# pyamg/pyamg

Measured on AMD Instinct MI355X. Metric: vcycle_iterations_per_sec, higher is better.
Workload: dtype f64; 1 GPU; 3D 7-pt Poisson 256^3 (16.7M dof) SA V-cycle, symmetric Gauss-Seidel, fp64; key=c3, n=16777216, nnz=117047296, levels=5, cycle=V(1,1), graph=True, parallelism=1 GPU, gs_order=fast, full=False

## Files before the change

include/pyamg_amd.h:

```cpp
#ifndef PYAMG_AMD_H
#define PYAMG_AMD_H

#include <stddef.h>
#include <stdint.h>

#ifdef __cplusplus
extern "C" {
#endif

#define PAMG_OK              0
#define PAMG_E_ARG          -1
#define PAMG_E_UNSUPPORTED  -2
#define PAMG_E_NODEVICE     -3
#define PAMG_E_STATE        -4
#define PAMG_E_ALLOC        -5
#define PAMG_E_TIMEOUT      -6
#define PAMG_E_NOCONV       -8

#define PAMG_F64 0
#define PAMG_F32 1

typedef void *pamg_stream_t;
typedef void *pamg_event_t;
typedef struct pamg_matrix_s *pamg_matrix_t;
// ... 314 lines not shown
#define PAMG_TUNE_ZERO_MERGE 40
#define PAMG_TUNE_GS_CORRECTION 41
int pamg_matrix_tune(pamg_matrix_t A, int key, int value);
int pamg_matrix_value_codes(pamg_matrix_t A, int *n_values);
int pamg_matrix_row_patterns(pamg_matrix_t A, int *n_patterns);
int pamg_matrix_row_masks(pamg_matrix_t A, long long info[8]);
int pamg_matrix_autotune(pamg_matrix_t A, int allow_cap);
int pamg_matrix_gs_profile(pamg_matrix_t A, int which, long long *out, int64_t capacity, int64_t *count);
int pamg_matrix_tile_info(pamg_matrix_t A, int which, int64_t info[8]);
int pamg_matrix_lane_info(pamg_matrix_t A, int which, int64_t info[8]);
int pamg_matrix_lanem_info(pamg_matrix_t A, int which, int64_t info[20], double *growth);
int pamg_matrix_point_twin(pamg_matrix_t A, int *state);
int pamg_matrix_lanem_levels(pamg_matrix_t A, int which, int64_t *out, int64_t capacity, int64_t *count);
int pamg_matrix_kz_info(pamg_matrix_t A, int which, int64_t info[8]);
int pamg_matrix_line_info(pamg_matrix_t A, int which, int64_t info[8]);
int pamg_matrix_lane_profile(pamg_matrix_t A, int which, long long *out, int64_t capacity, int64_t *count);
int pamg_matrix_subset_rows(pamg_matrix_t A, const int32_t *rows, int nrows, pamg_matrix_t *sub);
int pamg_matrix_kaczmarz(pamg_matrix_t L, int nr, void *v, const void *b, const void *Dinv, double omega,
                         int sweep, int iterations, void *xout, pamg_stream_t s);
int pamg_matrix_jacobi_indexed(pamg_matrix_t sub, void *x, const void *b, double omega, void *work,
                               pamg_stream_t s);
int pamg_matrix_flow_error(pamg_matrix_t A, int *error);

#define PAMG_SPMV_SET      0
#define PAMG_SPMV_ACC      1
#define PAMG_SPMV_RESID    2
#define PAMG_SPMV_AXPBY    3
#define PAMG_SPMV_ACC_AXPBY 4
int pamg_matrix_spmv(pamg_matrix_t A, int mode, const void *x, const void *b_or_v, double c,
                     void *y, pamg_stream_t s);
int pamg_matrix_split_ranges(pamg_matrix_t A, int64_t n_owned_cols);
int pamg_matrix_spmv_part(pamg_matrix_t A, int part, int mode, const void *x, const void *b_or_v, double c, void *y,
                          pamg_stream_t stream);
int pamg_matrix_resid_sumsq(pamg_matrix_t A, const void *x, const void *b, double *out_sumsq,
                            pamg_stream_t s);

#define PAMG_FORWARD   0
#define PAMG_BACKWARD  1
#define PAMG_SYMMETRIC 2
int pamg_matrix_jacobi(pamg_matrix_t A, void *x, const void *b, void *work, double omega,
                       int iterations, pamg_stream_t s);
int pamg_matrix_jacobi_step(pamg_matrix_t A, const void *x_in, const void *b, void *x_out,
                            double omega, pamg_stream_t s);
int pamg_matrix_block_jacobi_step(pamg_matrix_t A, const void *Dinv, const void *x_in, const void *b, void *x_out,
                                  double omega, pamg_stream_t s);
int pamg_matrix_block_jacobi_indexed(pamg_matrix_t A, const void *Dinv, void *x, const void *b, const int32_t *idx,
                                     int64_t nidx, double omega, void *work, pamg_stream_t s);
int pamg_matrix_gauss_seidel(pamg_matrix_t A, void *x, const void *b, int sweep, double omega,
                             int iterations, pamg_stream_t s);
int pamg_matrix_gauss_seidel_x0(pamg_matrix_t A, void *x, const void *b, int sweep, double omega,
                                int iterations, int x_is_zero, pamg_stream_t s);
int pamg_matrix_sym_info(pamg_matrix_t A, int64_t info[9]);
int pamg_matrix_gauss_seidel_correction(pamg_matrix_t A, void *x, const void *b, void *r, int iterations, pamg_stream_t s);
int pamg_matrix_polynomial(pamg_matrix_t A, void *x, const void *b, void *work,
                           const double *coeffs, int ncoeffs, int iterations, int x_is_zero,
                           pamg_stream_t s);
int pamg_matrix_block_jacobi(pamg_matrix_t A, void *x, const void *b, void *work,
                             const void *Dinv, double omega, int iterations, pamg_stream_t s);
int pamg_matrix_block_gauss_seidel(pamg_matrix_t A, void *x, const void *b, const void *Dinv,
                                   int sweep, int iterations, pamg_stream_t s);

int pamg_dev_pinv_array(int dtype, void *AA, int64_t m, int n, int transA, pamg_stream_t s);

int pamg_dev_schwarz_blocks(int dtype, pamg_matrix_t A, int nsub, const int32_t *d_Sp, const int32_t *d_Sj, int32_t *d_Tp,
                            void *d_Tx, int64_t Tx_capacity, double rank_tol, int invert, pamg_stream_t s, int64_t info[4]);
int pamg_schwarz_blocks(int dtype, pamg_matrix_t A, int nsub, const int32_t *Sp, const int32_t *Sj, int32_t *Tp, void *Tx,
                        int64_t Tx_capacity, double rank_tol, int invert, int64_t info[4]);

int pamg_vec_sumsq(int dtype, int64_t n, const void *x, double *out_sumsq, pamg_stream_t s);
int pamg_vec_axpy(int dtype, int64_t n, double a, const void *x, void *y, pamg_stream_t s);
int pamg_vec_scale(int dtype, int64_t n, double a, const void *x, void *y, pamg_stream_t s);
int pamg_vec_mul(int dtype, int64_t n, const void *a, const void *b, void *y, pamg_stream_t s);
int pamg_vec_gather(int dtype, int64_t n, const int32_t *idx, const void *src, void *dst,
                    pamg_stream_t s);

int pamg_csr_renumber(int dtype, int64_t nrows, int64_t ncols, const int32_t *Ap, const int32_t *Aj, const void *Ax,
                      const int32_t *row_old_of_new, const int32_t *col_new_of_old, int32_t *Bp, int32_t *Bj, void *Bx);
int pamg_csr_row_argmax_abs(int dtype, int64_t nrows, const int32_t *Ap, const int32_t *Aj, const void *Ax, int32_t *out);
int pamg_csr_sort_rows(int dtype, int64_t nrows, const int32_t *Ap, int32_t *Aj, void *Ax, int block);
int pamg_host_cpus(int fresh);

#define PAMG_SMOOTH_NONE        0
#define PAMG_SMOOTH_JACOBI      1
#define PAMG_SMOOTH_GS          2
#define PAMG_SMOOTH_SOR         3
#define PAMG_SMOOTH_POLY        4
#define PAMG_SMOOTH_BLOCK_JACOBI 5
#define PAMG_SMOOTH_BLOCK_GS    6
#define PAMG_SMOOTH_CF_JACOBI   7
#define PAMG_SMOOTH_FC_JACOBI   8
#define PAMG_SMOOTH_GS_NE       9
#define PAMG_SMOOTH_GS_NR      10
#define PAMG_SMOOTH_JACOBI_NE  11
#define PAMG_SMOOTH_CF_BLOCK_JACOBI 12
#define PAMG_SMOOTH_FC_BLOCK_JACOBI 13
#define PAMG_SMOOTH_SCHWARZ    14
#define PAMG_SMOOTH_KRYLOV     15
#define PAMG_KRYLOV_CG    0
#define PAMG_KRYLOV_GMRES 1
#define PAMG_KRYLOV_CGNE  2
#define PAMG_KRYLOV_CGNR  3
#define PAMG_CYCLE_V 0
#define PAMG_CYCLE_W 1
#define PAMG_CYCLE_F 2
#define PAMG_CYCLE_AMLI 3
int pamg_solver_create(pamg_solver_t *S, int dtype);
// ... 121 lines not shown
```

pyamg_amd/_build.py:

```python
from __future__ import annotations

import os
import shutil
import subprocess
import sys
from concurrent.futures import ThreadPoolExecutor
from pathlib import Path

PKG = Path(__file__).resolve().parent
CSRC = PKG / "csrc"
LIB = PKG / "libpyamg_amd.so"
SOURCES = ["pamg_matrix.hip", "pamg_solver.hip", "pamg_capi.hip", "pamg_setup.hip", "pamg_schwarz.hip", "pamg_dist.hip", "pamg_aggregate.hip", "pamg_lane.hip", "pamg_line.hip", "pamg_kz.hip", "pamg_blane.hip", "pamg_block.hip", "pamg_renumber.hip", "pamg_krylov.hip", "pamg_schwarz_setup.hip", "pamg_classical.hip", "pamg_air.hip", "pamg_evolution.hip", "pamg_energy.hip"]
HEADERS = ["pamg_common.h", "pamg_kernels.h", "pamg_tile_kernels.h", "pamg_tile_plan.h", "pamg_lane_plan.h", "pamg_lanem_plan.h", "pamg_schwarz_plan.h", "pamg_line_plan.h", "pamg_kz_plan.h", "pamg_blane_plan.h", "pamg_spg_plan.h", "pamg_stream_plan.h", "pamg_rowmask_map.h", "pamg_plan_vec.h", "pamg_host_threads.h", "pamg_dense_pinv.h", "pamg_classical.h", "pamg_air.h", "pamg_jacobi_svd.h", "pamg_evolution.h", "pamg_energy.h", "pamg_host_call.h", "pamg_wave.h", "pamg_sweep_host.h", "amg_core_bind.cpp", "../../include/pyamg_amd.h"]
FLAGS = ["--offload-arch=gfx950", "-O3", "-std=c++17", "-fPIC", "-ffp-contract=off",
         "-fno-fast-math", "-Wall", "-Wno-unused-function", "-Wno-unused-value", "-Wno-unused-result"]


def hipcc() -> str:
    for c in (os.environ.get("HIPCC"), shutil.which("hipcc"), "/opt/rocm/bin/hipcc"):
        if c and Path(c).exists():
            return c
    raise RuntimeError("hipcc not found (need ROCm's hipcc to build libpyamg_amd.so)")


def stale() -> bool:
    if not LIB.exists():
        return True
    try:
        import pybind11
        if shutil.which("g++") and not pybind_path().exists():
            return True
    except Exception:
        pass
    t = LIB.stat().st_mtime
    deps = [CSRC / s for s in SOURCES] + [(CSRC / h).resolve() for h in HEADERS] + [Path(__file__)]
    return any(d.stat().st_mtime > t for d in deps)


def build(force: bool = False, verbose: bool = True) -> Path:
    if not force and not stale():
        return LIB
    cc = hipcc()
    objdir = PKG / "build"
    objdir.mkdir(exist_ok=True)

    def one(src: str) -> Path:
        obj = objdir / (src + ".o")
        cmd = [cc, *FLAGS, "-c", str(CSRC / src), "-o", str(obj)]
        if verbose:
            print("[build]", " ".join(cmd), flush=True)
        subprocess.run(cmd, check=True)
        return obj

    with ThreadPoolExecutor(max_workers=len(SOURCES)) as ex:
        objs = list(ex.map(one, SOURCES))
    cmd = [cc, "--offload-arch=gfx950", "-shared", "-fPIC", *map(str, objs), "-o", str(LIB)]
    if verbose:
        print("[build]", " ".join(cmd), flush=True)
    subprocess.run(cmd, check=True)
    build_pybind(verbose)
    return LIB


def pybind_path() -> Path:
    import sysconfig
    return PKG / ("_amg_core_pybind" + (sysconfig.get_config_var("EXT_SUFFIX") or ".so"))
# ... 25 lines not shown
```

pyamg_amd/_capi.py:

```python
from __future__ import annotations

import ctypes as C
import os
from pathlib import Path

import numpy as np

PKG = Path(__file__).resolve().parent
LIB_PATH = Path(os.environ.get("PAMG_LIB", PKG / "libpyamg_amd.so"))

OK = 0
E_ARG, E_UNSUPPORTED, E_NODEVICE, E_STATE, E_ALLOC = -1, -2, -3, -4, -5
E_TIMEOUT, E_COMM, E_NOCONV = -6, -7, -8
F64, F32 = 0, 1
CSR, BSR = 0, 1
SPMV_SET, SPMV_ACC, SPMV_RESID, SPMV_AXPBY, SPMV_ACC_AXPBY = 0, 1, 2, 3, 4
FORWARD, BACKWARD, SYMMETRIC = 0, 1, 2
SMOOTH = {"schwarz": 14, "cf_block_jacobi": 12, "fc_block_jacobi": 13, "gauss_seidel_ne": 9, "gauss_seidel_nr": 10, "jacobi_ne": 11, "cf_jacobi": 7, "fc_jacobi": 8, "none": 0, "jacobi": 1, "gauss_seidel": 2, "sor": 3, "polynomial": 4,
          "block_jacobi": 5, "block_gauss_seidel": 6}
KRYLOV = {"cg": 0, "gmres": 1, "cgne": 2, "cgnr": 3}
ACCEL = {"bicgstab": 0, "cr": 1, "steepest_descent": 2, "minimal_residual": 3}
SWEEP = {"forward": FORWARD, "backward": BACKWARD, "symmetric": SYMMETRIC}
CYCLE = {"V": 0, "W": 1, "F": 2, "AMLI": 3}

# ... 104 lines not shown
    f("pamg_evolution_strength_vector_f64", *(_vp, _i) * 3, _i, *(_vp, _i) * 2)
    f("pamg_incomplete_mat_mult_bsr_f64", *(_vp, _i) * 9, _i, _i, _i, _i, _i)
    f("pamg_satisfy_constraints_helper_f64", _i, _i, _i, _i, *(_vp, _i) * 6)
    f("pamg_satisfy_constraints_f64", _i, _i, _i, _i, *(_vp, _i) * 5)
    f("pamg_energy_cg_f64", _i, _i, _i, _i, _i, _vp, _i, _vp, _i, _vp, C.c_int64, _vp, _i, _vp, _i, _vp, C.c_int64, _vp, _i, _vp, C.c_int64,
      _vp, _i, _vp, _vp, _i, _d, P(_i), _vp, P(_i))
    f("pamg_energy_gmres_f64", _i, _i, _i, _i, _i, _vp, _i, _vp, _i, _vp, C.c_int64, _vp, _i, _vp, _i, _vp, C.c_int64, _vp, _i, _vp, C.c_int64,
      _vp, _i, _vp, _vp, _i, _d, P(_i), _vp, P(_i), _vp)
    f("pamg_fit_tentative_f64", _i, _i, _i, _i, _vp, _vp, _vp, _vp, _vp, _d)
    f("pamg_fit_tentative_f32", _i, _i, _i, _i, _vp, _vp, _vp, _vp, _vp, C.c_float)
    f("pamg_matrix_create", P(_vp), _i, _i, _i, _i, _i, _i, _vp, _vp, _vp)
    f("pamg_matrix_destroy", _vp)
    f("pamg_matrix_info", _vp, P(C.c_int64))
    f("pamg_matrix_tune", _vp, _i, _i)
    f("pamg_matrix_value_codes", _vp, P(C.c_int))
    f("pamg_matrix_row_patterns", _vp, P(C.c_int))
    f("pamg_matrix_row_masks", _vp, P(C.c_longlong))
    f("pamg_matrix_flow_error", _vp, P(_i))
    f("pamg_matrix_subset_rows", _vp, _vp, _i, P(_vp))
    f("pamg_matrix_kaczmarz", _vp, _i, _vp, _vp, _vp, _d, _i, _i, _vp, _vp)
    f("pamg_vec_mul", _i, C.c_int64, _vp, _vp, _vp, _vp)
    f("pamg_matrix_jacobi_indexed", _vp, _vp, _vp, _d, _vp, _vp)
    f("pamg_matrix_gs_profile", _vp, _i, _vp, C.c_int64, P(C.c_int64))
    f("pamg_matrix_tile_info", _vp, _i, P(C.c_int64))
    f("pamg_matrix_lane_info", _vp, _i, P(C.c_int64))
    f("pamg_matrix_lanem_info", _vp, _i, P(C.c_int64), P(C.c_double))
    f("pamg_matrix_point_twin", _vp, P(_i))
    f("pamg_matrix_lanem_levels", _vp, _i, _vp, C.c_int64, P(C.c_int64))
    f("pamg_matrix_kz_info", _vp, _i, P(C.c_int64))
    f("pamg_matrix_line_info", _vp, _i, P(C.c_int64))
    f("pamg_matrix_lane_profile", _vp, _i, _vp, C.c_int64, P(C.c_int64))
    f("pamg_matrix_autotune", _vp, _i)
    f("pamg_matrix_spmv", _vp, _i, _vp, _vp, _d, _vp, _vp)
    f("pamg_matrix_split_ranges", _vp, C.c_int64)
    f("pamg_matrix_spmv_part", _vp, _i, _i, _vp, _vp, _d, _vp, _vp)
    f("pamg_matrix_resid_sumsq", _vp, _vp, _vp, _vp, _vp)
    f("pamg_matrix_jacobi", _vp, _vp, _vp, _vp, _d, _i, _vp)
    f("pamg_l1_cache_clear")
    f("pamg_l1_cache_size", P(C.c_int))
    f("pamg_matrix_jacobi_step", _vp, _vp, _vp, _vp, _d, _vp)
    f("pamg_matrix_block_jacobi_step", _vp, _vp, _vp, _vp, _vp, _d, _vp)
    f("pamg_matrix_block_jacobi_indexed", _vp, _vp, _vp, _vp, _vp, C.c_int64, _d, _vp, _vp)
    f("pamg_schwarz_create", P(_vp), _vp, _i, _vp, _vp, _vp, _vp)
    f("pamg_schwarz_destroy", _vp)
    f("pamg_schwarz_sweep", _vp, _vp, _vp, _i, _i, _i, _vp)
    f("pamg_schwarz_info", _vp, P(C.c_int64))
    f("pamg_schwarz_set_mode", _vp, _i)
    f("pamg_schwarz_error", _vp, P(_i))
    f("pamg_solver_set_schwarz_smoother", _vp, _i, _i, _i, _i, _vp, _i, _vp, _vp, _vp, _vp)
    f("pamg_solver_set_cf_block_smoother", _vp, _i, _i, _i, _i, _i, _i, _d, _vp, _i, _vp, _i, _vp, _i)
    f("pamg_matrix_gauss_seidel", _vp, _vp, _vp, _i, _d, _i, _vp)
    f("pamg_matrix_gauss_seidel_x0", _vp, _vp, _vp, _i, _d, _i, _i, _vp)
    f("pamg_matrix_gauss_seidel_correction", _vp, _vp, _vp, _vp, _i, _vp)
    f("pamg_matrix_sym_info", _vp, P(C.c_int64))
    f("pamg_matrix_polynomial", _vp, _vp, _vp, _vp, _vp, _i, _i, _i, _vp)
    f("pamg_matrix_block_jacobi", _vp, _vp, _vp, _vp, _vp, _d, _i, _vp)
    f("pamg_matrix_block_gauss_seidel", _vp, _vp, _vp, _vp, _i, _i, _vp)
    f("pamg_vec_sumsq", _i, C.c_int64, _vp, _vp, _vp)
    f("pamg_vec_axpy", _i, C.c_int64, _d, _vp, _vp, _vp)
    f("pamg_vec_scale", _i, C.c_int64, _d, _vp, _vp, _vp)
    f("pamg_vec_gather", _i, C.c_int64, _vp, _vp, _vp, _vp)
    f("pamg_csr_renumber", _i, C.c_int64, C.c_int64, _vp, _vp, _vp, _vp, _vp, _vp, _vp, _vp)
    f("pamg_csr_row_argmax_abs", _i, C.c_int64, _vp, _vp, _vp, _vp)
    f("pamg_csr_sort_rows", _i, C.c_int64, _vp, _vp, _vp, _i)
    f("pamg_host_cpus", _i)
    f("pamg_solver_create", P(_vp), _i)
    f("pamg_solver_destroy", _vp)
    f("pamg_solver_add_level", _vp, _vp, _vp, _vp)
    f("pamg_solver_set_smoother", _vp, _i, _i, _i, _i, _d, _i, _vp, _i, _vp, _i)
    f("pamg_solver_set_ne_smoother", _vp, _i, _i, _i, _i, _d, _i, _vp, _vp, _vp)
    f("pamg_solver_set_krylov_smoother", _vp, _i, _i, _i, _d, _i, _i, _vp)
    f("pamg_solver_set_cf_smoother", _vp, _i, _i, _i, _i, _i, _i, _d, _vp, _i, _vp, _i)
    f("pamg_solver_set_coarse_dense", _vp, _vp, _i)
    f("pamg_solver_set_coarse_relax", _vp)
    f("pamg_solver_set_coarse_host", _vp, _vp, _vp, _i)
    f("pamg_solver_finalize", _vp)
    f("pamg_solver_cycle", _vp, _vp, _vp, _i, _i, _vp)
    f("pamg_solver_solve", _vp, _vp, _vp, _d, _i, _i, _i, _i, _vp, P(_i), P(_i), _vp)
    f("pamg_solver_set_graph", _vp, _i)
    f("pamg_solver_pcg", _vp, _vp, _vp, _d, _i, _i, _i, _vp, P(_i), P(_i), _vp)
    f("pamg_solver_fgmres", _vp, _vp, _vp, _d, _i, _i, _i, _i, _vp, _i, P(_i), P(_i), P(_i), _vp)
    f("pamg_solver_gmres", _vp, _vp, _vp, _d, _i, _i, _i, _i, _vp, _i, P(_i), P(_i), P(_i), _vp)
    f("pamg_solver_krylov", _vp, _i, _vp, _vp, _d, _i, _i, _i, _vp, _i, P(_i), P(_i), P(_i), _vp)
    f("pamg_solver_load", _vp, _vp, _vp, _vp)
    f("pamg_solver_iterate", _vp, _i, _i, _i, _vp, _vp)
    f("pamg_solver_store", _vp, _vp, _vp)
    f("pamg_solver_stream", _vp, P(_vp))
    f("pamg_solver_stats", _vp, P(C.c_int64))
    f("pamg_dist_create", P(_vp), _i, _i, _i)
    f("pamg_dist_destroy", _vp)
    f("pamg_dist_add_level", _vp, _vp, _vp, _vp, C.c_int64, C.c_int64, _i, _vp, _vp, _vp, _i, _vp, _vp)
    f("pamg_dist_set_collapse", _vp, _vp, C.c_int64, C.c_int64, C.c_int64, C.c_int64, _vp)
    f("pamg_dist_set_smoother", _vp, _i, _i, _i, _i, _d, _vp, _i, _vp, _i)
    f("pamg_dist_set_callbacks", _vp, _vp, _vp, _vp)
    f("pamg_dist_rccl_unique_id", _vp)
    f("pamg_dist_set_rccl", _vp, _vp)
    f("pamg_dist_finalize", _vp)
    f("pamg_dist_set_options", _vp, _i, _i)
    f("pamg_dist_load", _vp, _vp, _vp)
    f("pamg_dist_store", _vp, _vp)
    f("pamg_dist_iterate", _vp, _i, _vp)
    f("pamg_dist_resid_norm", _vp, P(_d))
    f("pamg_dist_sync", _vp)
    f("pamg_dist_stream", _vp, P(_vp))
    f("pamg_dist_info", _vp, P(C.c_int64))
    f("pamg_dist_set_allgather", _vp, _i, C.c_int64, _vp)
# ... 152 lines not shown
```

pyamg_amd/csrc/pamg_common.h:

```cpp
#pragma once
#include "pamg_host_threads.h"
#include <hip/hip_runtime.h>

#include <cstdint>
#include <cstdio>
#include <cstdlib>
#include <ctime>
#include <algorithm>
#include <atomic>
#include <cstring>
#include <thread>
#include <vector>

#include "../../include/pyamg_amd.h"

#define PAMG_STR2(x) #x
#define PAMG_STR(x) PAMG_STR2(x)
#define PAMG_HIP(expr)                                   \
    do {                                                 \
        hipError_t e__ = (expr);                         \
        if (e__ != hipSuccess) return (int)e__;          \
    } while (0)
#define PAMG_TRY(expr)                                   \
    do {                                                 \
// ... 54 lines not shown
    int4 wb;
    const int *blkmap;
    const unsigned char *Ax8;
    const T *vdict;
    int nvd;
    const unsigned char *pid;
    const void *ptab;
    int npat, lmax;
};

struct GsSchedule {
    int row_start = 0, row_stop = 0, row_step = 0;
    int nlevels = 0;
    int64_t nrows = 0, nnz = 0;
    int *d_Ap = nullptr, *d_Aj = nullptr, *d_rid = nullptr;
    int4 *d_blkmeta = nullptr;
    void *d_Ax = nullptr, *d_diag = nullptr;
    int *d_level_blk = nullptr;
    int *d_pblk = nullptr;
    int *d_dpos = nullptr;
    void *d_xs = nullptr;
    void *d_xold = nullptr;
    long long *d_prof = nullptr;
    bool symmetric = false;
    int nblk_total = 0;
    unsigned *d_sync = nullptr;
    int max_level_blocks = 0;
    int max_range_rows = 0, max_range_blocks = 0;
    std::vector<int> level_blk;
    size_t bytes = 0;
    std::vector<int> h_vis, h_lvl;
    bool has_level_part = false;
    int cap = 0;
    struct TileSched *tile = nullptr;
    bool tile_unfit = false;
    struct LineSched *line = nullptr;
    bool line_unfit = false;
    struct LaneSched *lane = nullptr;
    bool lane_unfit = false;
    struct LaneMSched *lanem = nullptr;
    bool lanem_unfit = false;
    struct BlaneSched *blane = nullptr;
    bool blane_unfit = false;
};

struct TileSched {
    int G = 0, W = 0, NCH = 1, NV = 1, wide = 0, xo = 0, D = 0, Q = 0, nsteps = 0, lds = 0;
    unsigned char *d_blocks = nullptr;
    int *d_tile_step = nullptr;
    long long *d_prof = nullptr;
    int64_t n_local = 0, n_global = 0, n_publish = 0, max_step_entries = 0;
    size_t bytes = 0;
};

struct LineSchedule {
    int start = 0, stop = 0, step = 0;
    int nlevels = 0;
    int *d_lines = nullptr;
    int *d_level_ptr = nullptr;
    int *d_len = nullptr, *d_lo = nullptr, *d_ej = nullptr;
    void *d_ea = nullptr;
    std::vector<int> level_ptr;
    size_t bytes = 0;
    struct KzLaneSched *kzl = nullptr;
    bool kzl_unfit = false;
};

}

struct pamg_matrix_s {
    int dtype = PAMG_F64;
    int flavour = PAMG_CSR;
    int n_brow = 0, n_bcol = 0, R = 1, C = 1;
    int64_t nrows = 0, ncols = 0, nnz = 0;
    int *d_Ap = nullptr, *d_Aj = nullptr;
    void *d_Ax = nullptr;
    void *d_diag = nullptr;
    int *d_rowid = nullptr;
    int *d_bAp = nullptr, *d_bAj = nullptr;
    int *d_bAjf = nullptr, *d_bdiag = nullptr;
    void *d_bAx = nullptr;
    int64_t nblocks_b = 0;
    int4 *d_bmeta = nullptr;
    int bnblk = 0;
    std::vector<int> h_Ap, h_Aj;
    std::vector<int> h_bAp, h_bAj;
    int cap = 1536, max_rows = 1024;
    int flow_cap = 32;
    unsigned short *d_Aj16 = nullptr;
    int4 *d_wbase = nullptr;
    int use_idx16 = 1;
    unsigned char *d_Ax8 = nullptr;
    void *d_vdict = nullptr;
    int nvdict = 0;
    int use_val8 = 1;
    int use_rowg = 0;
    unsigned char *d_pid = nullptr;
    void *d_ptab = nullptr;
    int npat = 0, pat_lmax = 0;
    unsigned char *d_pmask = nullptr;
    int rm_nu = 0, rm_off[8] = {0, 0, 0, 0, 0, 0, 0, 0};
    unsigned long long rm_val[8] = {0, 0, 0, 0, 0, 0, 0, 0};
    long long rm_walked = 0;
    int rowmask_kz = 8;
    int rowmask_flags = 3;
    int use_rowpat = 1;
// ... 4 lines not shown
    int gran_cap = 0;
    int gs_mode = 0;
    int tile_G = 0;
    int tile_W = 0;
    int tile_cap = 0;
    int tile_D = 0, tile_Q = -1;
    int tile_part = 1;
    int tile_default = 0;
    int max_row_len = 0;
    int borrowed = 0;
    int gs_prof = 0;
    int gs_order = 0;
    int lane_L = 0, lane_G = 0;
    int lane_flags = 1;
    int line_scan = 1;
    int lane_merge = 0;
    int lanem_rpw = 0;
    int lanem_cluster = 0;
    int lanem_ahead10 = 40;
    int lane_wide = 0;
    int gs_cap = 0;
    int nblk = 0;
    int *d_part[2] = {nullptr, nullptr};
    int npart[2] = {0, 0};
    int64_t part_cols = -1;
    int64_t part_row0[2] = {-1, -1}, part_row1[2] = {-1, -1};
    int4 *d_blkmeta = nullptr;
    double *d_partial = nullptr;
    pamg::GsSchedule *gs[4] = {nullptr, nullptr, nullptr, nullptr};
    pamg_matrix_s *point_twin = nullptr;
    size_t point_twin_bytes = 0;
    bool point_twin_unfit = false;
    pamg::LineSchedule *ls[4] = {nullptr, nullptr, nullptr, nullptr};
    int sym_fused = 1;
    void *d_sym_hf[2] = {nullptr, nullptr}, *d_sym_hb = nullptr;
    unsigned *d_sym_sync = nullptr;
    int sym_cap = 0;
    const void *sym_cap_kernel = nullptr;
    int zsym_cap = 0;
    const void *zsym_cap_kernel = nullptr;
    int csym_cap = 0;
    const void *csym_cap_kernel = nullptr;
    int sym_general_grid = 0;
    int sym_form = 0, sym_grid = 0;
    long long sym_launches = 0, sym_zero_launches = 0;
    int zero_plans = 0;
    int zero_merge = 0;
    struct pamg::LaneMSched *zplan[2] = {nullptr, nullptr};
    void *d_zw = nullptr;
    size_t zero_bytes = 0;
    long long zero_plan_launches = 0;
    int gs_correction = 0;
    long long correction_launches = 0;
    size_t bytes = 0;
};

struct pamg_schwarz_s;
struct pamg_solver_s;
struct pamg_csr_s;

namespace pamg {
int schwarz_sweep(pamg_schwarz_s *h, void *x, const void *b, int start, int stop, int step, hipStream_t s);
int schwarz_prepare(pamg_schwarz_s *h, int sweep);
int schwarz_error(pamg_schwarz_s *h, bool *error);
void schwarz_level_launches(pamg_schwarz_s *h);
int schwarz_blocks_device(int dtype, pamg_matrix_s *A, int nsub, const int *d_Sp, const int *d_Sj, int *d_Tp, void *d_Tx,
                          int64_t Tx_capacity, double rank_tol, int invert, bool tp_given, hipStream_t s, int64_t info[4]);
int stream_launch(pamg_matrix_s *A, int epi, const void *x, const void *b, void *y, double c,
                  double omega, double *partial, hipStream_t s);
int stream_launch_part(pamg_matrix_s *A, int part, int epi, const void *x, const void *b, void *y, double c,
                       double omega, double *partial, hipStream_t s);
int matrix_split_ranges(pamg_matrix_s *A, int64_t n_owned_cols);
void matrix_drop_value_codes(pamg_matrix_s *A);
void matrix_drop_point_twin(pamg_matrix_s *A);
void matrix_drop_schedules(pamg_matrix_s *A);
int gs_sweep(pamg_matrix_s *A, int epi, void *x, const void *b, double omega, int row_start,
             int row_stop, int row_step, hipStream_t s);
int gs_sweep_symmetric(pamg_matrix_s *A, void *x, const void *b, bool x_zero, hipStream_t s, bool *ran);
int ensure_sym_parts(pamg_matrix_s *A);
int sym_reset(pamg_matrix_s *A);
int reduce_partials(const double *partial, int n, double *out, hipStream_t s);
int vec_sumsq(int dtype, int64_t n, const void *x, double *scratch, double *out, hipStream_t s);
int vec_axpy(int dtype, int64_t n, double a, const void *x, void *y, hipStream_t s);
int vec_scale(int dtype, int64_t n, double a, const void *x, void *y, hipStream_t s);
int vec_dot(int dtype, int64_t n, const void *x, const void *y, double *scratch, double *out, hipStream_t s);
int vec_mul(int dtype, int64_t n, const void *a, const void *b, void *y, hipStream_t s);
int kaczmarz_sweep(pamg_matrix_s *L, bool nr, void *v, const void *b, const void *Dinv, double omega, int start, int stop,
                   int step, void *xout, hipStream_t s);
int ensure_line_schedule(pamg_matrix_s *L, int start, int stop, int step);
void free_line_schedule(LineSchedule *g);
int vec_scatter(int dtype, int64_t n, const int *idx, const void *src, void *dst, hipStream_t s);
int vec_copy_indexed(int dtype, int64_t n, const int *idx, const void *src, void *dst, hipStream_t s);
int matrix_row_subset(pamg_matrix_s *A, const int32_t *rows, int nrows, pamg_matrix_s **out);
int jacobi_indexed(pamg_matrix_s *sub, void *x, const void *b, double omega, void *work, hipStream_t s);
int vec_maxratio(int dtype, int64_t n, const void *u, const void *x, double *scratch, double *out, hipStream_t s);
int vec_xpby(int dtype, int64_t n, double beta, const void *z, void *p, hipStream_t s);
int vec_axpy_ratio(int dtype, int64_t n, const double *num, const double *den, double sign, const void *x, void *y, hipStream_t s);
int vec_fill(int dtype, int64_t n, double v, void *y, hipStream_t s);
int dense_gemv(int dtype, int n, const void *M, const void *b, void *x, hipStream_t s);
int block_gs_sweep(pamg_matrix_s *A, void *x, const void *b, const void *Dinv, int row_start,
                   int row_stop, int row_step, hipStream_t s);
int block_jacobi_step(pamg_matrix_s *A, int kind, const void *Dinv, const void *xsrc, void *xdst,
                      const void *b, double omega, hipStream_t s);
int ensure_schedule(pamg_matrix_s *A, int row_start, int row_stop, int row_step, bool block_gs = false);
struct CsrArrays { int64_t m, n, nnz; const int *p, *j; const double *x; };
int csr_device_arrays(struct ::pamg_csr_s *A, CsrArrays *out);
// ... 17 lines not shown
              hipStream_t s);
int kr_take(int dtype, int64_t n, void *xc, void *dst, double *part, hipStream_t s);
int solver_cycle_inline(pamg_solver_s *S, void *x, const void *b, int cycle, int cpl, hipStream_t s, bool allow_graph);
bool solver_needs_host_sync(const pamg_solver_s *S);
bool line_eligible(const pamg_matrix_s *A, const GsSchedule *g);
int build_line_part(pamg_matrix_s *A, GsSchedule *g);
void free_line_part(LineSched *t);
size_t line_part_bytes(const GsSchedule *g);
int line_launch(pamg_matrix_s *A, GsSchedule *g, int epi, void *x, const void *b, double omega, hipStream_t s);
int line_info(const GsSchedule *g, int64_t *info);
int line_sym_launch(pamg_matrix_s *A, GsSchedule *gf, GsSchedule *gb, void *x, const void *b, hipStream_t s);
int build_kz_lane_part(pamg_matrix_s *Lm, LineSchedule *g);
void free_kz_lane_part(KzLaneSched *t);
int kz_lane_launch(pamg_matrix_s *Lm, LineSchedule *g, bool nr, void *v, const void *b, const void *Dinv, double omega, void *xout, hipStream_t s);
int kz_lane_info(const LineSchedule *g, int64_t *info);
bool kz_lane_error(LineSchedule *g);
bool want_blanes(const pamg_matrix_s *A, const GsSchedule *g);
int block_point_sweep(pamg_matrix_s *A, GsSchedule *g, void *x, const void *b, int dirn, hipStream_t s);
int get_schedule(pamg_matrix_s *A, int row_start, int row_stop, int row_step, GsSchedule **out);
int ensure_parts(pamg_matrix_s *A, GsSchedule *g, bool block_gs = false);
int device_cus();
bool blane_eligible(const pamg_matrix_s *A, const GsSchedule *g);
int build_blane_part(pamg_matrix_s *A, GsSchedule *g);
void free_blane_part(BlaneSched *t);
size_t blane_part_bytes(const GsSchedule *g);
int blane_launch(pamg_matrix_s *A, GsSchedule *g, const void *Dinv, void *x, const void *b, hipStream_t s);
int blane_info(const GsSchedule *g, int64_t *info);
int blane_profile(const GsSchedule *g, long long *out, int64_t cap, int64_t *n);
bool lane_eligible(const pamg_matrix_s *A, const GsSchedule *g);
int build_lane_part(pamg_matrix_s *A, GsSchedule *g);
void free_lane_part(LaneSched *t);
size_t lane_part_bytes(const GsSchedule *g);
int lane_launch(pamg_matrix_s *A, GsSchedule *g, int epi, void *x, const void *b, double omega, hipStream_t s);
int lane_info(const GsSchedule *g, int64_t *info);
int lane_profile(const GsSchedule *g, long long *out, int64_t cap, int64_t *n);
int lanem_smax(const pamg_matrix_s *A, const GsSchedule *g);
int build_lanem_part(pamg_matrix_s *A, GsSchedule *g);
void free_lanem_part(struct LaneMSched *t);
size_t lanem_part_bytes(const GsSchedule *g);
int lanem_info(const GsSchedule *g, int64_t *info, double *growth);
int lanem_levels(const GsSchedule *g, int64_t *out, int64_t cap, int64_t *n);
int lanem_sym_launch(pamg_matrix_s *A, GsSchedule *gf, GsSchedule *gb, void *x, const void *b, bool x_zero, hipStream_t s, bool acc = false);
int lanem_plan_info(const struct LaneMSched *t, int64_t *info, double *growth);
int build_zero_plan(pamg_matrix_s *A, int dir);
void free_zero_plans(pamg_matrix_s *A);
size_t zero_plan_bytes(const pamg_matrix_s *A);
bool zero_plans_ready(const pamg_matrix_s *A, const GsSchedule *gf, const GsSchedule *gb);
int lanem_zero_pair_launch(pamg_matrix_s *A, GsSchedule *gf, GsSchedule *gb, void *x, const void *b, bool acc, hipStream_t s);
int ensure_zero_parts(pamg_matrix_s *A, bool build);
void matrix_drop_zero_plans(pamg_matrix_s *A);
int gs_sweep_zero_pair(pamg_matrix_s *A, void *x, const void *b, hipStream_t s, bool *ran);
int gs_sweep_correction(pamg_matrix_s *A, void *x, const void *b, void *r, bool force, hipStream_t s, bool *ran);
constexpr int64_t GS_CORRECTION_MIN_ROWS = 16384;
int sym_fill_sentinels(void *p, int64_t n);
int sweep_error(pamg_matrix_s *A, bool *error);
inline size_t tsize(int dtype) { return dtype == PAMG_F64 ? 8 : 4; }

template <typename F>
inline void host_parallel(int64_t n, F fn, int64_t grain = 1 << 20)
{
    const unsigned hw = std::max(1u, std::min(32u, pamg::host_cpus()));
    const int nt = n < 2 * grain ? 1 : (int)std::min<int64_t>(hw, n / grain);
    if (nt <= 1) { fn((int64_t)0, n); return; }
    std::vector<std::thread> th;
    for (int t = 0; t < nt; ++t) {
        const int64_t lo = n * t / nt, hi = n * (t + 1) / nt;
        th.emplace_back([=] { fn(lo, hi); });
    }
    for (auto &x : th) x.join();
}

struct PhaseTimer {
    const char *name;
    int64_t items;
    timespec t0;
    static bool on() { static const int v = [] { const char *e = getenv("PAMG_TIMING"); return (e && *e && *e != '0') ? 1 : 0; }(); return v != 0; }
    explicit PhaseTimer(const char *n, int64_t k = 0) : name(n), items(k) { if (on()) clock_gettime(CLOCK_MONOTONIC, &t0); }
    ~PhaseTimer()
    {
        if (!on()) return;
        timespec t1;
        clock_gettime(CLOCK_MONOTONIC, &t1);
        fprintf(stderr, "[pamg timing] %-28s %8.3f s  (%lld)\n", name, (double)(t1.tv_sec - t0.tv_sec) + 1e-9 * (double)(t1.tv_nsec - t0.tv_nsec), (long long)items);
    }
};
}
```

pyamg_amd/csrc/pamg_lane.hip:

```cpp
#include "pamg_common.h"
#include "pamg_lane_plan.h"
#include "pamg_lanem_plan.h"
#include "pamg_tile_plan.h"
#include "pamg_wave.h"
#include "pamg_sweep_host.h"

namespace pamg {

struct alignas(16) LaneRec { int rid; int gate; int rd_lo; int rd_hi; };

struct LaneSched {
    int L = 0, K = 0, RPW = 0;
    int64_t ngroups = 0;
    int *d_cols = nullptr;
    LaneRec *d_rec = nullptr;
    void *d_vals = nullptr;
    long long *d_prof = nullptr;
    int64_t n_early = 0, n_old = 0, n_slots = 0;
    int64_t max_level_groups = 0;
    int last_grid = 0;
    int cap = 0;
    const void *cap_kernel = nullptr;
    size_t bytes = 0;
};
// ... 1103 lines not shown
{
    for (int d = 0; d < 2; ++d) { free_lanem_part(A->zplan[d]); A->zplan[d] = nullptr; }
    hipFree(A->d_zw);
    A->d_zw = nullptr;
}

size_t zero_plan_bytes(const pamg_matrix_s *A)
{
    size_t b = A->d_zw ? ((size_t)A->nrows + 8) * sizeof(double) : 0;
    for (int d = 0; d < 2; ++d) if (A->zplan[d]) b += A->zplan[d]->bytes;
    return b;
}

bool zero_plans_ready(const pamg_matrix_s *A, const GsSchedule *gf, const GsSchedule *gb)
{
    const LaneMSched *zf = A->zplan[0], *zb = A->zplan[1];
    if (A->zero_plans == 1 || !zf || !zb || !A->d_zw || !gf || !gb || !gf->lanem || !gb->lanem) return false;
    return zf->rpw == zb->rpw && zf->cluster == zb->cluster && zf->rpw == gf->lanem->rpw && zf->cluster == gf->lanem->cluster &&
           zb->rpw == gb->lanem->rpw && zb->cluster == gb->lanem->cluster && zf->ngroups >= 1 && zb->ngroups >= 1;
}

static void lanem_layout_args(const LaneMSched *t, LaneMArgs &a)
{
    a.cols = t->d_cols; a.vals = t->d_vals;
    a.rec = t->cluster ? reinterpret_cast<const LaneMRec *>(t->d_crec) : t->d_rec;
    a.sidx = t->d_sidx; a.crid = t->d_crid; a.crd = t->d_crd; a.crows = t->cluster;
}

template <int Z>
static const void *lanem_kernel(int cluster, int rpw, bool all_regs, bool xcd)
{
    if (cluster) return (const void *)gs_lanem_kernel<0, 0, 8, Z>;
    if (rpw == 2) return xcd ? (const void *)gs_lanem_kernel<1, 2, 4, Z> : (const void *)gs_lanem_kernel<0, 2, 4, Z>;
    if (all_regs) return xcd ? (const void *)gs_lanem_kernel<1, 1, 8, Z> : (const void *)gs_lanem_kernel<0, 1, 8, Z>;
    return xcd ? (const void *)gs_lanem_kernel<1, 1, 2, Z> : (const void *)gs_lanem_kernel<0, 1, 2, Z>;
}
template <int Z>
static const void *lanem_sym_kernel(int cluster, int rpw, bool all_regs, bool xcd)
{
    if (cluster) return (const void *)gs_lanem_sym_kernel<0, 0, 8, Z>;
    if (rpw == 2) return xcd ? (const void *)gs_lanem_sym_kernel<1, 2, 4, Z> : (const void *)gs_lanem_sym_kernel<0, 2, 4, Z>;
    if (all_regs) return xcd ? (const void *)gs_lanem_sym_kernel<1, 1, 8, Z> : (const void *)gs_lanem_sym_kernel<0, 1, 8, Z>;
    return xcd ? (const void *)gs_lanem_sym_kernel<1, 1, 2, Z> : (const void *)gs_lanem_sym_kernel<0, 1, 2, Z>;
}

static bool lanem_all_regs(const pamg_matrix_s *A, const LaneMSched *t)
{
    static const int nreg_env = [] { const char *e = getenv("PAMG_LANEM_NREG"); return e ? atoi(e) : 0; }();
    return t->rpw == 1 && (nreg_env ? nreg_env == 8 : A->nrows <= 131072);
}

static bool lanem_one_xcd(const pamg_matrix_s *A, const GsSchedule *g, const LaneMSched *t)
{
    return !t->cluster && (A->gran_xcd == 1 || (A->gran_xcd == 0 && lane_one_xcd(A, g) && A->nrows <= 8192));
}

static int lanem_want_grid(const pamg_matrix_s *A, const LaneMSched *t, int cap, int cus)
{
    const int per_level = (int)((t->ngroups + t->nsuper - 1) / std::max(1, t->nsuper));
    const int64_t want_waves = std::max<int64_t>(128, ((int64_t)A->lanem_ahead10 * per_level + 9) / 10);
    int G = (int)std::min<int64_t>((want_waves + LANE_WPB - 1) / LANE_WPB, (int64_t)std::min(cap, (t->rpw == 2 || t->cluster) ? 2 : 3) * cus);
    if (A->lane_G > 0) G = std::min(A->lane_G, cap * cus);
    return (int)std::max<int64_t>(1, std::min<int64_t>(G, (t->ngroups + LANE_WPB - 1) / LANE_WPB));
}

static int lanem_launch_plan(pamg_matrix_s *A, GsSchedule *g, LaneMSched *t, void *x, const void *b, double *w, hipStream_t s, bool acc = false)
{
    if (!t || !g->d_xold) return PAMG_E_STATE;
    const int64_t n = A->nrows;
    LaneMArgs a;
    lanem_layout_args(t, a);
    a.use_gate = (A->lane_flags & 1) ? 1 : 0;
    a.xold = (const double *)g->d_xold; a.y = (double *)x; a.xs = (double *)g->d_xs; a.b = (const double *)b;
    a.w = w;
    a.err = g->d_sync + 1; a.ticket = g->d_sync + 20;
    a.ngroups = (int)t->ngroups;
    a.nidle = (int)std::max<int64_t>(1, std::min<int64_t>(n, 1 << 20));
    if (A->gs_prof && !t->cluster) PAMG_TRY(ensure_profile(&t->d_prof, t->ngroups));
    a.prof = (A->gs_prof && !t->cluster) ? t->d_prof : nullptr;
    const int fgrid = (int)std::min<int64_t>(4096, (n + BLK - 1) / BLK);
    if (acc) hipLaunchKernelGGL((fill_sentinel_kernel<double>), dim3(fgrid), dim3(BLK), 0, s, (double *)g->d_xs, n);
    else hipLaunchKernelGGL(lanem_prepare_kernel, dim3(fgrid), dim3(BLK), 0, s, (const double *)x, (double *)g->d_xold, (double *)g->d_xs, n);
    PAMG_HIP(hipGetLastError());
    const bool xcd = lanem_one_xcd(A, g, t);
    const bool all_regs = lanem_all_regs(A, t);
    const int Z = acc ? 2 : w ? 1 : 0;
    const void *k = Z == 0 ? lanem_kernel<0>(t->cluster, t->rpw, all_regs, xcd)
                  : Z == 1 ? lanem_kernel<1>(t->cluster, t->rpw, all_regs, xcd)
                           : lanem_kernel<2>(t->cluster, t->rpw, all_regs, xcd);
    const int cus = device_cus();
    const int cap = resident_cap(t->cap, t->cap_kernel, k);
    void *args[] = {(void *)&a};
    return launch_persistent(k, args, lanem_want_grid(A, t, cap, cus), xcd, g->d_sync + 20, cus, cap, &t->last_grid, s);
}

int lanem_launch(pamg_matrix_s *A, GsSchedule *g, void *x, const void *b, hipStream_t s) { return lanem_launch_plan(A, g, g->lanem, x, b, nullptr, s); }

int lanem_zero_pair_launch(pamg_matrix_s *A, GsSchedule *gf, GsSchedule *gb, void *x, const void *b, bool acc, hipStream_t s)
{
    if (!zero_plans_ready(A, gf, gb)) return PAMG_E_UNSUPPORTED;
    if (acc) {
        if (!gb->d_xold) return PAMG_E_STATE;
        PAMG_HIP(hipMemsetAsync(gb->d_xold, 0, (size_t)A->nrows * sizeof(double), s));
        PAMG_TRY(lanem_launch_plan(A, gf, A->zplan[0], gb->d_xold, b, (double *)A->d_zw, s));
        PAMG_TRY(lanem_launch_plan(A, gb, A->zplan[1], x, A->d_zw, nullptr, s, true));
    } else {
        PAMG_TRY(lanem_launch_plan(A, gf, A->zplan[0], x, b, (double *)A->d_zw, s));
// ... 163 lines not shown
```

pyamg_amd/csrc/pamg_matrix.hip:

```cpp
#include "pamg_host_threads.h"
#include <algorithm>
#include <atomic>
#include <mutex>
#include <climits>
#include <new>
#include <thread>

#include "pamg_kernels.h"
#include "pamg_tile_kernels.h"
#include "pamg_tile_plan.h"
#include "pamg_stream_plan.h"

using namespace pamg;

namespace {

constexpr int PAD = 8;

std::mutex g_sched_mu;

template <typename U>
int upload(U **dptr, const U *h, size_t n, size_t *bytes)
{
    const size_t sz = (n + PAD) * sizeof(U);
    PAMG_HIP(hipMalloc((void **)dptr, sz));
    PAMG_HIP(hipMemset(*dptr, 0, sz));
    if (n) PAMG_HIP(hipMemcpy(*dptr, h, n * sizeof(U), hipMemcpyHostToDevice));
    if (bytes) *bytes += sz;
    return PAMG_OK;
}

int upload_raw(void **dptr, const void *h, size_t n, size_t elt, size_t *bytes)
{
    const size_t sz = (n + PAD) * elt;
    PAMG_HIP(hipMalloc(dptr, sz));
    PAMG_HIP(hipMemset(*dptr, 0, sz));
    if (n) PAMG_HIP(hipMemcpy(*dptr, h, n * elt, hipMemcpyHostToDevice));
    if (bytes) *bytes += sz;
    return PAMG_OK;
}

void plan_rows(const int *Ap, int begin, int end, int cap, int max_rows, std::vector<int4> &out)
{
    std::vector<RowRange> rr;
    plan_row_ranges(Ap, begin, end, cap, max_rows, rr);
    for (const RowRange &q : rr) out.push_back(make_int4(q.r0, q.r1, q.p0, q.p1));
}

int lds_bytes(int dtype, int epi, int cap)
{
    const int per = (int)tsize(dtype) + ((epi == EPI_JACOBI || epi == EPI_JACOBI_B || epi == EPI_JACOBI_IDX) ? 4 : 0);
    return per * (cap + 8) + 64;
}

int val8_lds(const pamg_matrix_s *A, int epi)
{
    const int per = (int)tsize(A->dtype) + ((epi == EPI_JACOBI || epi == EPI_JACOBI_B || epi == EPI_JACOBI_IDX) ? 4 : 0);
    return 8 * per + 16 + (int)tsize(A->dtype) * ((A->nvdict + 1) & ~1);
}

template <typename T, int EPI>
int launch_epi(int grid, int lds, hipStream_t s, const StreamArgs<T> &a)
{
    if (grid <= 0) return PAMG_OK;
// ... 705 lines not shown
    a.wbase = nullptr;
    a.wb = make_int4(0, 0, 0, 0);
    a.blkmap = nullptr;
    a.Ax8 = nullptr;
    a.vdict = nullptr;
    a.nvd = 0;
    a.pid = nullptr;
    a.ptab = nullptr;
    a.npat = a.lmax = 0;
    return a;
}

double *g_scratch = nullptr;
int g_scratch_dev = -1;

}

namespace pamg {

void matrix_drop_value_codes(pamg_matrix_s *A) { if (A) drop_val8(A); }

void matrix_drop_point_twin(pamg_matrix_s *A)
{
    if (!A) return;
    pamg_matrix_s *T = nullptr;
    {
        std::lock_guard<std::mutex> lk(g_sched_mu);
        T = A->point_twin;
        if (T) A->bytes -= std::min(A->bytes, A->point_twin_bytes);
        A->point_twin = nullptr;
        A->point_twin_bytes = 0;
        A->point_twin_unfit = false;
    }
    if (T) pamg_matrix_destroy(T);
}

void matrix_drop_schedules(pamg_matrix_s *A)
{
    if (!A) return;
    for (int k = 0; k < 4; ++k) {
        GsSchedule *g = nullptr;
        LineSchedule *l = nullptr;
        {
            std::lock_guard<std::mutex> lk(g_sched_mu);
            g = A->gs[k]; l = A->ls[k];
            if (g) A->bytes -= std::min(A->bytes, g->bytes);
            if (l) A->bytes -= std::min(A->bytes, l->bytes);
            A->gs[k] = nullptr; A->ls[k] = nullptr;
        }
        free_schedule(g);
        if (l) free_line_schedule(l);
    }
    matrix_drop_zero_plans(A);
    matrix_drop_point_twin(A);
}

int matrix_split_ranges(pamg_matrix_s *A, int64_t n_owned_cols)
{
    if (!A || n_owned_cols < 0) return PAMG_E_ARG;
    for (int k = 0; k < 2; ++k) { if (A->d_part[k]) { hipFree(A->d_part[k]); A->d_part[k] = nullptr; } A->npart[k] = 0; A->part_row0[k] = A->part_row1[k] = -1; }
    A->part_cols = -1;
    if (A->nblk == 0 || A->h_Ap.empty()) { A->part_cols = n_owned_cols; return PAMG_OK; }
    std::vector<int4> blk;
    blk.reserve((size_t)A->nblk);
    plan_rows(A->h_Ap.data(), 0, (int)A->nrows, A->cap, A->max_rows, blk);
    if ((int)blk.size() != A->nblk) return PAMG_E_STATE;
    std::vector<unsigned char> bnd(blk.size(), 0);
    const int *Aj = A->h_Aj.data();
    const int lim = (int)std::min<int64_t>(n_owned_cols, INT_MAX);
    parallel_rows((int)blk.size(), [&](int lo, int hi) {
        for (int b = lo; b < hi; ++b) {
            unsigned char any = 0;
            for (int p = blk[b].z; p < blk[b].w && !any; ++p) any = Aj[p] >= lim;
            bnd[(size_t)b] = any;
        }
    });
    std::vector<int> part[2];
    for (int b = 0; b < (int)blk.size(); ++b) part[bnd[(size_t)b] ? 1 : 0].push_back(b);
    for (int k = 0; k < 2; ++k) {
        A->npart[k] = (int)part[k].size();
        PAMG_TRY(upload(&A->d_part[k], part[k].data(), part[k].size(), &A->bytes));
        A->part_row0[k] = A->part_row1[k] = -1;
        if (!part[k].empty() && part[k].back() - part[k].front() + 1 == (int)part[k].size()) {
            A->part_row0[k] = blk[(size_t)part[k].front()].x;
            A->part_row1[k] = blk[(size_t)part[k].back()].y;
        }
    }
    A->part_cols = n_owned_cols;
    return PAMG_OK;
}

int stream_launch(pamg_matrix_s *A, int epi, const void *x, const void *b, void *y, double c,
                  double omega, double *partial, hipStream_t s)
{
    return stream_launch_part(A, 0, epi, x, b, y, c, omega, partial, s);
}

int stream_launch_part(pamg_matrix_s *A, int part, int epi, const void *x, const void *b, void *y, double c,
                       double omega, double *partial, hipStream_t s)
{
    if (part < 0 || part > 2) return PAMG_E_ARG;
    if (part && A->part_cols < 0) return PAMG_E_STATE;
    if (part) {
        const int n = A->npart[part - 1];
        if (n == 0) return PAMG_OK;
        const bool idx16 = A->use_idx16 && A->d_Aj16;
// ... 509 lines not shown
    A->bytes -= std::min(A->bytes, A->zero_bytes);
    A->zero_bytes = zero_plan_bytes(A);
    A->bytes += A->zero_bytes;
    return PAMG_OK;
}

int gs_sweep_zero_pair(pamg_matrix_s *A, void *x, const void *b, hipStream_t s, bool *ran)
{
    *ran = false;
    if (A->zero_plans == 1 || (A->zero_plans == 0 && !A->zplan[0])) return PAMG_OK;
    GsSchedule *gf = nullptr, *gb = nullptr;
    if (!zero_form_of(A, &gf, &gb)) return PAMG_OK;
    if (!zero_plans_ready(A, gf, gb)) {
        if (A->zero_plans != 2 || A->zplan[0] || A->zplan[1]) return PAMG_OK;
        hipStreamCaptureStatus cs = hipStreamCaptureStatusNone;
        PAMG_HIP(hipStreamIsCapturing(s, &cs));
        if (cs != hipStreamCaptureStatusNone) return PAMG_OK;
        PAMG_TRY(ensure_zero_parts(A, true));
        if (!zero_plans_ready(A, gf, gb)) { A->zero_plans = 1; return PAMG_OK; }
    }
    const int st = lanem_zero_pair_launch(A, gf, gb, x, b, false, s);
    if (st == PAMG_E_UNSUPPORTED) return PAMG_OK;
    if (st == PAMG_OK) *ran = true;
    return st;
}

int gs_sweep_correction(pamg_matrix_s *A, void *x, const void *b, void *r, bool force, hipStream_t s, bool *ran)
{
    *ran = false;
    if (!r || A->zero_plans == 1) return PAMG_OK;
    if (!force && (A->gs_correction == 1 || (A->gs_correction == 0 && A->nrows < GS_CORRECTION_MIN_ROWS))) return PAMG_OK;
    if (!A->zplan[0] || !A->zplan[1] || !A->d_zw) {
        if (!force || A->zero_plans != 2 || A->zplan[0] || A->zplan[1]) return PAMG_OK;
        hipStreamCaptureStatus cs = hipStreamCaptureStatusNone;
        PAMG_HIP(hipStreamIsCapturing(s, &cs));
        if (cs != hipStreamCaptureStatusNone) return PAMG_OK;
        PAMG_TRY(ensure_zero_parts(A, true));
    }
    GsSchedule *gf = nullptr, *gb = nullptr;
    if (!zero_form_of(A, &gf, &gb) || !zero_plans_ready(A, gf, gb)) return PAMG_OK;
    GsSchedule *sf = nullptr, *sb = nullptr;
    bool fused = sym_form_of(A, &sf, &sb) == 1;
    if (fused && !A->d_sym_hf[0]) {
        hipStreamCaptureStatus cs = hipStreamCaptureStatusNone;
        PAMG_HIP(hipStreamIsCapturing(s, &cs));
        if (cs == hipStreamCaptureStatusNone) PAMG_TRY(ensure_sym_parts(A));
        fused = A->d_sym_hf[0] != nullptr;
    }
    PAMG_TRY(stream_launch(A, EPI_RESID, x, b, r, 0.0, 0.0, nullptr, s));
    int st = fused ? lanem_sym_launch(A, gf, gb, x, r, true, s, true) : PAMG_E_UNSUPPORTED;
    if (st == PAMG_E_UNSUPPORTED) st = lanem_zero_pair_launch(A, gf, gb, x, r, true, s);
    if (st != PAMG_OK) return st;
    A->correction_launches++;
    *ran = true;
    return PAMG_OK;
}

int ensure_schedule(pamg_matrix_s *A, int row_start, int row_stop, int row_step, bool block_gs)
{
    GsSchedule *g = nullptr;
    PAMG_TRY(get_schedule(A, row_start, row_stop, row_step, &g));
    return ensure_parts(A, g, block_gs);
}

int reduce_partials(const double *partial, int n, double *out, hipStream_t s)
{
    if (n > 8192) {
        double *mid = const_cast<double *>(partial) + n;
        hipLaunchKernelGGL(reduce_mid_kernel, dim3(256), dim3(BLK), 0, s, partial, n, mid);
        hipLaunchKernelGGL(reduce_final_kernel, dim3(1), dim3(BLK), 0, s, (const double *)mid, 256, out);
    } else {
        hipLaunchKernelGGL(reduce_final_kernel, dim3(1), dim3(BLK), 0, s, partial, n, out);
    }
    return (int)hipGetLastError();
}

int vec_sumsq(int dtype, int64_t n, const void *x, double *scratch, double *out, hipStream_t s)
{
    const int grid = (int)std::min<int64_t>(1024, std::max<int64_t>(1, (n + BLK - 1) / BLK));
    if (dtype == PAMG_F64)
        hipLaunchKernelGGL((vec_sumsq_kernel<double>), dim3(grid), dim3(BLK), 0, s, (const double *)x, n, scratch);
    else
        hipLaunchKernelGGL((vec_sumsq_kernel<float>), dim3(grid), dim3(BLK), 0, s, (const float *)x, n, scratch);
    PAMG_HIP(hipGetLastError());
    return reduce_partials(scratch, grid, out, s);
}

int vec_dot(int dtype, int64_t n, const void *x, const void *y, double *scratch, double *out, hipStream_t s)
{
    const int grid = (int)std::min<int64_t>(1024, std::max<int64_t>(1, (n + BLK - 1) / BLK));
    if (dtype == PAMG_F64)
        hipLaunchKernelGGL((vec_dot_kernel<double>), dim3(grid), dim3(BLK), 0, s, (const double *)x, (const double *)y, n, scratch);
    else
        hipLaunchKernelGGL((vec_dot_kernel<float>), dim3(grid), dim3(BLK), 0, s, (const float *)x, (const float *)y, n, scratch);
    PAMG_HIP(hipGetLastError());
    hipLaunchKernelGGL(reduce_final_kernel, dim3(1), dim3(BLK), 0, s, (const double *)scratch, grid, out);
    return (int)hipGetLastError();
}

static int vgrid(int64_t n) { return (int)std::min<int64_t>(1 << 21, std::max<int64_t>(1, (n + BLK - 1) / BLK)); }

int vec_mul(int dtype, int64_t n, const void *a, const void *b, void *y, hipStream_t s)
{
    if (n <= 0) return PAMG_OK;
    const int grid = vgrid(n);
    if (dtype == PAMG_F64)
// ... 366 lines not shown
            A->h_bAj.assign(Aj, Aj + nblk);
            A->nblocks_b = nblk;
            st = upload(&A->d_bAp, A->h_bAp.data(), A->h_bAp.size(), &A->bytes);
            if (!st) st = upload(&A->d_bAj, A->h_bAj.data(), A->h_bAj.size(), &A->bytes);
            if (!st) st = upload_raw(&A->d_bAx, Ax, (size_t)A->nnz, ts, &A->bytes);
            std::vector<int> bjf(A->h_bAj), bdiag((size_t)n_brow, -1);
            for (int i = 0; i < n_brow; ++i)
                for (int p = Ap[i]; p < Ap[i + 1]; ++p)
                    if (Aj[p] == i) { bjf[p] = i | 0x40000000; bdiag[i] = p; }
            if (!st) st = upload(&A->d_bAjf, bjf.data(), bjf.size(), &A->bytes);
            if (!st) st = upload(&A->d_bdiag, bdiag.data(), bdiag.size(), &A->bytes);
        }
    }
    if (!st) {
        std::atomic<int> mx(0);
        host_parallel(A->nrows, [&](int64_t lo, int64_t hi) {
            int m = 0;
            for (int64_t i = lo; i < hi; ++i) m = std::max(m, A->h_Ap[i + 1] - A->h_Ap[i]);
            int cur = mx.load();
            while (m > cur && !mx.compare_exchange_weak(cur, m)) {}
        });
        A->max_row_len = mx.load();
    }
    A->cap = 1536; A->max_rows = 1024;
    if (A->d_Ax8 && R == 1 && C == 1) {
        const int64_t avg = (A->nnz + A->nrows - 1) / std::max<int64_t>(1, A->nrows);
        const int64_t rows = std::min<int64_t>(512, std::max<int64_t>(64, ((A->nrows / 2048 + 63) / 64) * 64));
        A->max_rows = (int)rows;
        A->cap = (int)std::min<int64_t>(12288, std::max<int64_t>(512, ((rows * avg + 255) / 256) * 256));
        A->cap_from_val8 = 1;
        A->use_rowg = 1;
    }
    if (!st) st = replan(A);
    if (!st && A->d_Ax8 && !A->d_Aj16) {
        drop_val8(A);
        A->cap = 1536; A->max_rows = 1024; A->cap_from_val8 = 0; A->use_rowg = 0;
        st = replan(A);
    }
    if (st) { pamg_matrix_destroy(A); return st; }
    *out = A;
    return PAMG_OK;
}

int pamg_matrix_destroy(pamg_matrix_t A)
{
    if (!A) return PAMG_OK;
    hipFree(A->d_Ap); hipFree(A->d_Aj); hipFree(A->d_Ax); hipFree(A->d_diag); hipFree(A->d_rowid);
    hipFree(A->d_bAp); hipFree(A->d_bAj); hipFree(A->d_bAjf); hipFree(A->d_bdiag); hipFree(A->d_bAx); hipFree(A->d_blkmeta); hipFree(A->d_partial); hipFree(A->d_bmeta); hipFree(A->d_Aj16); hipFree(A->d_wbase); hipFree(A->d_Ax8); hipFree(A->d_vdict); hipFree(A->d_pid); hipFree(A->d_ptab);
    hipFree(A->d_part[0]); hipFree(A->d_part[1]);
    for (int k = 0; k < 4; ++k) free_schedule(A->gs[k]);
    for (int k = 0; k < 4; ++k) pamg::free_line_schedule(A->ls[k]);
    hipFree(A->d_sym_hf[0]); hipFree(A->d_sym_hf[1]); hipFree(A->d_sym_hb); hipFree(A->d_sym_sync);
    pamg::free_zero_plans(A);
    if (A->point_twin) pamg_matrix_destroy(A->point_twin);
    delete A;
    return PAMG_OK;
}

int pamg_matrix_point_twin(pamg_matrix_t A, int *state)
{
    if (!A || !state) return PAMG_E_ARG;
    *state = A->point_twin_unfit ? 2 : A->point_twin ? 1 : 0;
    return PAMG_OK;
}

int pamg_matrix_info(pamg_matrix_t A, int64_t info[8])
{
    if (!A || !info) return PAMG_E_ARG;
    info[0] = A->nrows; info[1] = A->ncols; info[2] = A->nnz; info[3] = A->nblk;
    info[4] = A->cap; info[5] = (int64_t)A->bytes;
    info[6] = info[7] = 0;
    const int n = A->R > 1 ? A->n_brow : (int)A->nrows;
    for (int k = 0; k < 4; ++k) {
        GsSchedule *g = A->gs[k];
        if (!g) continue;
        if (g->row_start == 0 && g->row_stop == n && g->row_step == 1) info[6] = g->nlevels;
        if (g->row_start == n - 1 && g->row_stop == -1 && g->row_step == -1) info[7] = g->nlevels;
    }
    return PAMG_OK;
}

int pamg_matrix_value_codes(pamg_matrix_t A, int *n_values)
{
    if (!A || !n_values) return PAMG_E_ARG;
    *n_values = (A->d_Ax8 && A->use_val8 && A->use_idx16 && A->d_Aj16) ? A->nvdict : 0;
    return PAMG_OK;
}

int pamg_matrix_row_patterns(pamg_matrix_t A, int *n_patterns)
{
    if (!A || !n_patterns) return PAMG_E_ARG;
    *n_patterns = (A->d_pid && A->use_rowpat && A->d_Ax8 && A->use_val8 && A->use_idx16 && A->d_Aj16) ? A->npat : 0;
    return PAMG_OK;
}

int pamg_matrix_row_masks(pamg_matrix_t A, long long info[8])
{
    if (!A || !info) return PAMG_E_ARG;
    for (int k = 0; k < 8; ++k) info[k] = 0;
    int npat = 0;
    pamg_matrix_row_patterns(A, &npat);
    if (!npat || !A->d_pmask || (A->use_rowpat != 1 && A->use_rowpat != 4)) return PAMG_OK;
    info[0] = A->rm_nu; info[1] = A->rm_walked; info[5] = A->rowmask_kz; info[6] = A->rowmask_flags;
    info[7] = (A->nrows + BLK - 1) / BLK;
    RowMaskLattice g;
    int grid3 = 0;
// ... 60 lines not shown
    {PAMG_TUNE_ROWPAT,        &M::use_rowpat,    one_of<0, 1, 3, 4>,     KEEP,             AS_IS,   HELD_OK},
    {PAMG_TUNE_GS_ORDER,      &M::gs_order,      in<0, 1>,               KEEP,             AS_IS,   0},
    {PAMG_TUNE_LANE_L,        &M::lane_L,        one_of<0, 4, 8, 16, 32, 64>, DROP_LANES,  AS_IS,   TWIN},
    {PAMG_TUNE_LANE_G,        &M::lane_G,        in<0, INT_MAX>,         DROP_TWIN,        AS_IS,   TWIN},
    {PAMG_TUNE_LANE_WIDE,     &M::lane_wide,     in<0, 1>,               DROP_TWIN,        AS_IS,   TWIN},
    {PAMG_TUNE_LANE_FLAGS,    &M::lane_flags,    flags_in<0, 15, 6>,     DROP_TWIN,        AS_IS,   TWIN},
    {PAMG_TUNE_LINE_SCAN,     &M::line_scan,     in<0, 2>,               DROP_TWIN_LINE,   AS_IS,   TWIN},
    {PAMG_TUNE_ROWMASK_KZ,    &M::rowmask_kz,    one_of<2, 4, 8>,        KEEP,             AS_IS,   0},
    {PAMG_TUNE_ROWMASK_FLAGS, &M::rowmask_flags, in<0, 7>,               KEEP,             AS_IS,   0},
    {PAMG_TUNE_LANE_MERGE,    &M::lane_merge,    in<0, 8>,               DROP_LANES,       AS_IS,   TWIN},
    {PAMG_TUNE_LANEM_AHEAD,   &M::lanem_ahead10, in<1, 400>,             DROP_TWIN,        AS_IS,   TWIN},
    {PAMG_TUNE_LANEM_RPW,     &M::lanem_rpw,     in<0, 2>,               DROP_LANES,       AS_IS,   TWIN},
    {PAMG_TUNE_LDS_PAD,       &M::lds_pad,       in<0, 98304>,           KEEP,             ALIGN16, 0},
    {PAMG_TUNE_SYM_FUSED,     &M::sym_fused,     in<0, 1>,               KEEP,             AS_IS,   0},
    {PAMG_TUNE_LANEM_CLUSTER, &M::lanem_cluster, one_of<0, 1, 4, 8>,     DROP_LANES,       AS_IS,   TWIN},
    {PAMG_TUNE_ZERO_PLANS,    &M::zero_plans,    in<0, 2>,               DROP_ZERO_IF_OFF, AS_IS,   0},
    {PAMG_TUNE_ZERO_MERGE,    &M::zero_merge,    zero_or_in<2, 16>,      DROP_ZERO,        AS_IS,   0},
    {PAMG_TUNE_GS_CORRECTION, &M::gs_correction, in<0, 2>,               KEEP,             AS_IS,   0},
};

void tune_inherit(pamg_matrix_s *T, const pamg_matrix_s *A)
{
    for (const TuneKey &t : TUNE_KEYS) if (t.flags & TWIN) T->*(t.field) = A->*(t.field);
}

int tune_stored(TuneStore store, int value) { return store == NONZERO ? value != 0 : store == ALIGN4 ? (value & ~3) : store == ALIGN16 ? (value & ~15) : value; }

template <typename Part>
void drop_part(pamg_matrix_s *A, GsSchedule *g, Part *&part, size_t bytes, void (*free_part)(Part *))
{
    if (!part) return;
    A->bytes -= bytes; g->bytes -= bytes;
    free_part(part);
    part = nullptr;
}

int tune_effect(pamg_matrix_s *A, TuneEffect effect, int value)
{
    switch (effect) {
        case KEEP: return PAMG_OK;
        case DROP_ZERO_IF_OFF: if (value != 1) return PAMG_OK; [[fallthrough]];
        case DROP_ZERO: matrix_drop_zero_plans(A); return PAMG_OK;
        case DROP_TWIN_LINE:
            for (GsSchedule *g : A->gs) {
                if (!g) continue;
                g->line_unfit = false;
                if (value == 0) drop_part(A, g, g->line, line_part_bytes(g), free_line_part);
            }
            [[fallthrough]];
        case DROP_TWIN: matrix_drop_point_twin(A); return PAMG_OK;
        case DROP_LANES:
            matrix_drop_point_twin(A);
            matrix_drop_zero_plans(A);
            for (GsSchedule *g : A->gs) {
                if (!g) continue;
                g->lane_unfit = g->lanem_unfit = g->blane_unfit = g->line_unfit = false;
                drop_part(A, g, g->lane, lane_part_bytes(g), free_lane_part);
                drop_part(A, g, g->lanem, lanem_part_bytes(g), free_lanem_part);
                drop_part(A, g, g->blane, blane_part_bytes(g), free_blane_part);
            }
            return PAMG_OK;
        case DROP_TILES:
            for (GsSchedule *g : A->gs) {
                if (!g) continue;
                g->tile_unfit = false;
                drop_part(A, g, g->tile, g->tile ? g->tile->bytes : 0, free_tile_part);
            }
            return PAMG_OK;
        case REPLAN_WINDOW: A->cap_from_val8 = 0; [[fallthrough]];
        case REPLAN:
            for (int k = 0; k < 4; ++k) { if (A->gs[k]) A->bytes -= A->gs[k]->bytes; free_schedule(A->gs[k]); A->gs[k] = nullptr; }
            matrix_drop_zero_plans(A);
            matrix_drop_point_twin(A);
            return replan(A);
    }
    return PAMG_E_ARG;
}

}

extern "C" {

int pamg_matrix_tune(pamg_matrix_t A, int key, int value)
{
    if (!A) return PAMG_E_ARG;
    const TuneKey *t = std::find_if(std::begin(TUNE_KEYS), std::end(TUNE_KEYS), [key](const TuneKey &r) { return r.key == key; });
    if (t == std::end(TUNE_KEYS)) t = nullptr;
    if (A->borrowed > 0 && !(t && (t->flags & HELD_OK))) return PAMG_E_STATE;
    if (!t || !t->accepts(value)) return PAMG_E_ARG;
    A->*(t->field) = tune_stored(t->store, value);
    return tune_effect(A, t->effect, value);
}

int pamg_matrix_autotune(pamg_matrix_t A, int allow_cap)
{
    if (!A) return PAMG_E_ARG;
    if (A->borrowed > 0) return PAMG_E_STATE;
    if (A->nnz < 4000000) return PAMG_OK;
    const size_t ts = tsize(A->dtype);
    void *x = nullptr, *y = nullptr;
    PAMG_HIP(hipMalloc(&x, (size_t)(A->ncols + 8) * ts));
    if (hipMalloc(&y, (size_t)(A->nrows + 8) * ts) != hipSuccess) { hipFree(x); return (int)hipErrorOutOfMemory; }
    hipMemset(x, 0, (size_t)(A->ncols + 8) * ts);
    hipEvent_t e0, e1;
    hipEventCreate(&e0); hipEventCreate(&e1);
    const int cap0 = A->cap, fl0 = A->stream_flags;
    const int caps[2] = {cap0, 512};
    int best_cap = cap0, best_fl = fl0, st = PAMG_OK;
    float best_ms = 1e30f;
    long long rm0[8];
    const bool masked = pamg_matrix_row_masks(A, rm0) == PAMG_OK && rm0[0] > 0;
    const int idx0 = A->use_idx16;
    const int nidx = (A->d_Aj16 && !A->d_Ax8 && idx0) ? 2 : 1;
    const bool square = A->nrows == A->ncols;
    const int probe = square ? EPI_RESID : EPI_SET;
    void *pb = nullptr;
    if (square) {
        if (hipMalloc(&pb, (size_t)(A->nrows + 8) * ts) != hipSuccess) { hipFree(x); hipFree(y); hipEventDestroy(e0); hipEventDestroy(e1); return (int)hipErrorOutOfMemory; }
        hipMemset(pb, 0, (size_t)(A->nrows + 8) * ts);
    }
    float cand_ms[2][2][2][2];
    for (int q = 0; q < 16; ++q) (&cand_ms[0][0][0][0])[q] = 1e30f;
    const int nvc = A->d_Ax8 ? 1 : 2;
    for (int ci = 0; ci < (allow_cap ? 2 : 1) && st == PAMG_OK && !masked; ++ci) {
        if (caps[ci] != A->cap) { A->cap = caps[ci]; st = replan(A); if (st) break; }
        for (int round = 0; round < 2 && st == PAMG_OK; ++round) {
            for (int ix = 0; ix < nidx && st == PAMG_OK; ++ix) {
                A->use_idx16 = ix == 0 ? idx0 : 0;
                for (int fl = 0; fl < 2 && st == PAMG_OK; ++fl)
                    for (int vc = 0; vc < nvc && st == PAMG_OK; ++vc) {
                        A->stream_flags = (fl0 & ~(1 | 32)) | fl | (vc ? 32 : 0);
                        for (int w = 0; w < 2 && st == PAMG_OK; ++w) st = stream_launch(A, probe, x, pb, y, 0.0, 0.0, nullptr, nullptr);
                        hipEventRecord(e0, nullptr);
                        for (int r = 0; r < 6 && st == PAMG_OK; ++r) st = stream_launch(A, probe, x, pb, y, 0.0, 0.0, nullptr, nullptr);
                        hipEventRecord(e1, nullptr);
                        hipEventSynchronize(e1);
                        float ms = 0.f;
                        hipEventElapsedTime(&ms, e0, e1);
                        if (st == PAMG_OK) cand_ms[ci][ix][fl][vc] = std::min(cand_ms[ci][ix][fl][vc], ms);
                    }
            }
        }
    }
// ... 73 lines not shown
    for (int l = 0; l < g->nlevels; ++l)
        for (int q = g->level_blk[l]; q < g->level_blk[l + 1]; ++q) out[(size_t)q * 8 + 7] = l;
    return PAMG_OK;
}

int pamg_matrix_line_info(pamg_matrix_t A, int which, int64_t info[8])
{
    if (!A || which < 0 || which > 3 || !info) return PAMG_E_ARG;
    return pamg::line_info(A->gs[which], info);
}

int pamg_matrix_lane_info(pamg_matrix_t A, int which, int64_t info[8])
{
    if (!A || which < 0 || which > 3 || !info) return PAMG_E_ARG;
    if (A->R > 1) return pamg::blane_info(A->gs[which], info);
    return pamg::lane_info(A->gs[which], info);
}

int pamg_matrix_kz_info(pamg_matrix_t A, int which, int64_t info[8])
{
    if (!A || !info || which < 0 || which > 3) return PAMG_E_ARG;
    return pamg::kz_lane_info(A->ls[which], info);
}

int pamg_matrix_lanem_info(pamg_matrix_t A, int which, int64_t info[20], double *growth)
{
    if (!A || !info || which < 0 || which > 5) return PAMG_E_ARG;
    if (which >= 4) return pamg::lanem_plan_info(A->zplan[which - 4], info, growth);
    return pamg::lanem_info(A->gs[which], info, growth);
}

int pamg_matrix_sym_info(pamg_matrix_t A, int64_t info[9])
{
    if (!A || !info) return PAMG_E_ARG;
    for (int k = 0; k < 9; ++k) info[k] = 0;
    info[0] = A->sym_launches; info[1] = A->sym_zero_launches; info[2] = A->sym_form; info[3] = A->sym_general_grid ? A->sym_general_grid : A->sym_grid; info[4] = A->sym_fused;
    info[5] = -1; info[6] = -1;
    info[7] = A->zero_plan_launches;
    info[8] = A->correction_launches;
    if (!A->d_sym_hf[0]) return PAMG_OK;
    PAMG_HIP(hipDeviceSynchronize());
    unsigned w[8] = {0, 0, 0, 0, 0, 0, 0, 0};
    PAMG_HIP(hipMemcpy(w, A->d_sym_sync, sizeof(w), hipMemcpyDeviceToHost));
    std::vector<unsigned long long> h((size_t)A->nrows);
    if (A->nrows) PAMG_HIP(hipMemcpy(h.data(), A->d_sym_hf[w[5] & 1u], (size_t)A->nrows * 8, hipMemcpyDeviceToHost));
    int64_t bad = 0;
    for (unsigned long long v : h) bad += (v != pamg::Sentinel<double>::value);
    info[5] = bad;
    info[6] = 0;
    for (int k = 0; k < 5; ++k) info[6] += w[k] != 0u;
    return PAMG_OK;
}

int pamg_matrix_lanem_levels(pamg_matrix_t A, int which, int64_t *out, int64_t capacity, int64_t *count)
{
    if (!A || !count || which < 0 || which > 3) return PAMG_E_ARG;
    return pamg::lanem_levels(A->gs[which], out, capacity, count);
}

int pamg_matrix_lane_profile(pamg_matrix_t A, int which, long long *out, int64_t capacity, int64_t *count)
{
    if (!A || which < 0 || which > 3 || !count) return PAMG_E_ARG;
    PAMG_HIP(hipDeviceSynchronize());
    if (A->R > 1) return pamg::blane_profile(A->gs[which], out, capacity, count);
    return pamg::lane_profile(A->gs[which], out, capacity, count);
}

int pamg_matrix_tile_info(pamg_matrix_t A, int which, int64_t info[8])
{
    if (!A || which < 0 || which > 3 || !info) return PAMG_E_ARG;
    for (int k = 0; k < 8; ++k) info[k] = 0;
    const GsSchedule *g = A->gs[which];
    if (!g || !g->tile) return PAMG_OK;
    const TileSched *t = g->tile;
    info[0] = t->G; info[1] = t->W; info[2] = (t->NCH + t->NV + 1) | (t->D << 8) | (TILE_VAR[t->wide][2] << 16) | (t->Q << 24); info[3] = t->nsteps;
    info[4] = t->n_local; info[5] = t->n_global; info[6] = t->n_publish; info[7] = t->lds;
    return PAMG_OK;
}

int pamg_matrix_kaczmarz(pamg_matrix_t L, int nr, void *v, const void *b, const void *Dinv, double omega, int sweep,
                         int iterations, void *xout, pamg_stream_t s)
{
    if (!L || iterations < 0 || sweep < PAMG_FORWARD || sweep > PAMG_SYMMETRIC) return PAMG_E_ARG;
    const int n = (int)L->nrows;
    if (n == 0) return PAMG_OK;
    for (int it = 0; it < iterations; ++it) {
        if (sweep != PAMG_BACKWARD) PAMG_TRY(pamg::kaczmarz_sweep(L, nr != 0, v, b, Dinv, omega, 0, n, 1, xout, (hipStream_t)s));
        if (sweep != PAMG_FORWARD) PAMG_TRY(pamg::kaczmarz_sweep(L, nr != 0, v, b, Dinv, omega, n - 1, -1, -1, xout, (hipStream_t)s));
    }
    return PAMG_OK;
}

int pamg_vec_mul(int dtype, int64_t n, const void *a, const void *b, void *y, pamg_stream_t s)
{
    if (dtype != PAMG_F64 && dtype != PAMG_F32) return PAMG_E_ARG;
    return pamg::vec_mul(dtype, n, a, b, y, (hipStream_t)s);
}

int pamg_matrix_subset_rows(pamg_matrix_t A, const int32_t *rows, int nrows, pamg_matrix_t *sub)
{
    return pamg::matrix_row_subset(A, rows, nrows, sub);
}

int pamg_matrix_jacobi_indexed(pamg_matrix_t sub, void *x, const void *b, double omega, void *work, pamg_stream_t s)
{
    return pamg::jacobi_indexed(sub, x, b, omega, work, (hipStream_t)s);
// ... 98 lines not shown
```

pyamg_amd/csrc/pamg_solver.hip:

```cpp
#include <algorithm>
#include <cmath>
#include <functional>
#include <map>
#include <new>
#include <thread>

#include "pamg_common.h"

using namespace pamg;

namespace {

struct Smoother {
    int kind = PAMG_SMOOTH_NONE;
    int iterations = 1;
    double omega = 1.0;
    int sweep = PAMG_FORWARD;
    std::vector<double> coeffs;
    void *d_Dinv = nullptr;
    int blocksize = 1;
    pamg_matrix_s *AF = nullptr, *AC = nullptr;
    void *wF = nullptr, *wC = nullptr;
    int f_iterations = 1, c_iterations = 1;
    int *iF = nullptr, *iC = nullptr;
// ... 17 lines not shown

int sweep_bounds(const pamg_matrix_s *A, int dir, int &r0, int &r1, int &rs)
{
    const int n = A->R > 1 ? A->n_brow : (int)A->nrows;
    if (dir == PAMG_FORWARD) { r0 = 0; r1 = n; rs = 1; }
    else if (dir == PAMG_BACKWARD) { r0 = n - 1; r1 = -1; rs = -1; }
    else return PAMG_E_ARG;
    return PAMG_OK;
}

bool square_ok(const pamg_matrix_s *A) { return A && A->nrows == A->ncols && A->R == A->C; }

int jacobi_pp(pamg_matrix_s *A, void **px, void **palt, const void *b, double omega, int its, hipStream_t s)
{
    if (!square_ok(A)) return PAMG_E_ARG;
    if (A->nrows == 0) return PAMG_OK;
    for (int it = 0; it < its; ++it) {
        if (A->R > 1)
            PAMG_TRY(block_jacobi_step(A, PNT_JACOBI, nullptr, *px, *palt, b, omega, s));
        else
            PAMG_TRY(stream_launch(A, A->flavour == PAMG_BSR ? EPI_JACOBI_B : EPI_JACOBI, *px, b, *palt,
                                   0.0, omega, nullptr, s));
        std::swap(*px, *palt);
    }
    return PAMG_OK;
}

int block_jacobi_pp(pamg_matrix_s *A, void **px, void **palt, const void *b, const void *Dinv,
                    double omega, int its, hipStream_t s)
{
    if (!square_ok(A) || A->R < 2 || !Dinv) return PAMG_E_ARG;
    for (int it = 0; it < its; ++it) {
        PAMG_TRY(block_jacobi_step(A, BLK_JACOBI, Dinv, *px, *palt, b, omega, s));
        std::swap(*px, *palt);
    }
    return PAMG_OK;
}

int gs_apply(pamg_matrix_s *A, void *x, const void *b, int sweep, double omega, int its, hipStream_t s, bool x_zero = false, void *r = nullptr)
{
    if (!square_ok(A)) return PAMG_E_ARG;
    if (A->nrows == 0) return PAMG_OK;
    auto one = [&](int dir, double om) -> int {
        int r0, r1, rs;
        PAMG_TRY(sweep_bounds(A, dir, r0, r1, rs));
        int epi;
        if (A->R > 1 || A->flavour == PAMG_BSR) epi = EPI_GS_B;
        else epi = (om != 1.0) ? EPI_SOR : EPI_GS;
        return gs_sweep(A, epi, x, b, om, r0, r1, rs, s);
    };
    if (sweep == PAMG_SYMMETRIC) {
        for (int it = 0; it < its; ++it) {
            bool ran = false;
            if (r && !(x_zero && it == 0)) PAMG_TRY(gs_sweep_correction(A, x, b, r, false, s, &ran));
            if (ran) continue;
            PAMG_TRY(gs_sweep_symmetric(A, x, b, x_zero && it == 0, s, &ran));
            if (ran) continue;
            if (x_zero && it == 0) PAMG_TRY(gs_sweep_zero_pair(A, x, b, s, &ran));
            if (ran) continue;
            PAMG_TRY(one(PAMG_FORWARD, 1.0));
            PAMG_TRY(one(PAMG_BACKWARD, 1.0));
        }
        return PAMG_OK;
    }
    for (int it = 0; it < its; ++it) PAMG_TRY(one(sweep, omega));
    return PAMG_OK;
}

int block_gs_apply(pamg_matrix_s *A, void *x, const void *b, const void *Dinv, int sweep, int its,
                   hipStream_t s)
{
    if (!square_ok(A) || A->R < 2 || !Dinv) return PAMG_E_ARG;
    auto one = [&](int dir) -> int {
        int r0, r1, rs;
        PAMG_TRY(sweep_bounds(A, dir, r0, r1, rs));
        return block_gs_sweep(A, x, b, Dinv, r0, r1, rs, s);
    };
    for (int it = 0; it < its; ++it) {
        if (sweep == PAMG_SYMMETRIC) { PAMG_TRY(one(PAMG_FORWARD)); PAMG_TRY(one(PAMG_BACKWARD)); }
        else PAMG_TRY(one(sweep));
    }
    return PAMG_OK;
}

int poly_apply(pamg_matrix_s *A, void *x, const void *b, void *work, const double *coeffs, int nc,
               int its, int x_is_zero, hipStream_t s)
{
    if (!A || A->nrows != A->ncols || nc < 1 || !coeffs) return PAMG_E_ARG;
    const int64_t n = A->nrows;
    if (n == 0) return PAMG_OK;
    const size_t ts = tsize(A->dtype);
    void *res_buf = work, *h0 = (char *)work + n * ts, *h1 = (char *)work + 2 * n * ts;
    for (int it = 0; it < its; ++it) {
        const void *res = b;
        bool have_h = false;
        if (!(x_is_zero && it == 0)) {
            PAMG_TRY(stream_launch(A, EPI_RESID, x, b, res_buf, nc > 1 ? coeffs[0] : 0.0, 0.0, nc > 1 ? (double *)h0 : nullptr, s));
            res = res_buf;
            have_h = nc > 1;
        }
        if (nc == 1) {
            PAMG_TRY(vec_axpy(A->dtype, n, coeffs[0], res, x, s));
            continue;
        }
        if (!have_h) PAMG_TRY(vec_scale(A->dtype, n, coeffs[0], res, h0, s));
        void *hc = h0, *hn = h1;
// ... 113 lines not shown
                    const int reps = f ? sm.f_iterations : sm.c_iterations;
                    for (int k = 0; k < reps; ++k) {
                        PAMG_TRY(block_jacobi_step(L.A, BLK_JACOBI, sm.d_Dinv, L.x, L.xalt, L.b, sm.omega, s));
                        PAMG_TRY(vec_copy_indexed(S->dtype, f ? sm.nF : sm.nC, f ? sm.iF : sm.iC, L.xalt, L.x, s));
                    }
                }
            }
            return PAMG_OK;
    }
    (void)S;
    return PAMG_E_ARG;
}

void drop_graphs(pamg_solver_s *S);
int prebuild_schedules(Level &L, const Smoother &sm, bool zero = false);

int check_sweeps(pamg_solver_s *S)
{
    bool any = false;
    for (Level &L : S->levels) {
        if (!L.A) continue;
        bool e = false;
        PAMG_TRY(sweep_error(L.A, &e));
        any = any || e;
        for (Smoother *sm : {&L.pre, &L.post}) {
            for (pamg_matrix_s *M : {sm->At, sm->Ar})
                if (M && M != L.A) {
                    bool e2 = false;
                    PAMG_TRY(sweep_error(M, &e2));
                    any = any || e2;
                }
            if (sm->sw) {
                bool e3 = false;
                PAMG_TRY(schwarz_error(sm->sw, &e3));
                any = any || e3;
            }
        }
    }
    static int forced = [] { const char *e = getenv("PAMG_FORCE_TIMEOUT"); return e ? atoi(e) : 0; }();
    if (forced > 0) { --forced; any = true; }
    return any ? PAMG_E_TIMEOUT : PAMG_OK;
}

int fall_back_to_level_launches(pamg_solver_s *S)
{
    hipDeviceSynchronize();
    drop_graphs(S);
    for (Level &L : S->levels) {
        if (!L.A) continue;
        L.A->gs_mode = 1;
        L.A->tile_default = 0;
        PAMG_TRY(sym_reset(L.A));
        matrix_drop_zero_plans(L.A);
        for (Smoother *sm : {&L.pre, &L.post}) {
            if (sm->At) sm->At->gs_mode = 1;
            if (sm->Ar) sm->Ar->gs_mode = 1;
            if (sm->sw) schwarz_level_launches(sm->sw);
            PAMG_TRY(prebuild_schedules(L, *sm));
        }
    }
    S->fallbacks++;
    return PAMG_OK;
}

int coarse_solve(pamg_solver_s *S, const void *b, void *x, hipStream_t s)
{
    if (S->coarse_relax) {
        Level &L = S->levels.back();
        if (b != L.b || x != L.x) return PAMG_E_STATE;
        PAMG_HIP(hipMemsetAsync(L.x, 0, (size_t)L.n * tsize(S->dtype), s));
        PAMG_TRY(apply_smoother(S, L, L.pre, true, s));
        if (L.x != L.x_home) {
            PAMG_HIP(hipMemcpyAsync(L.x_home, L.x, (size_t)L.n * tsize(S->dtype), hipMemcpyDeviceToDevice, s));
            std::swap(L.x, L.xalt);
        }
        return PAMG_OK;
    }
    if (S->coarse_zero) return (int)hipMemsetAsync(x, 0, (size_t)S->n_c * tsize(S->dtype), s);
    if (S->coarse_host) {
        const size_t vb = (size_t)S->n_c * tsize(S->dtype);
        PAMG_HIP(hipMemcpyAsync(S->coarse_hb.data(), b, vb, hipMemcpyDeviceToHost, s));
        PAMG_HIP(hipStreamSynchronize(s));
        if (S->coarse_host(S->coarse_host_user, S->coarse_hb.data(), S->coarse_hx.data(), (int64_t)S->n_c) != 0) return PAMG_E_STATE;
        PAMG_HIP(hipMemcpyAsync(x, S->coarse_hx.data(), vb, hipMemcpyHostToDevice, s));
        PAMG_HIP(hipStreamSynchronize(s));
        return PAMG_OK;
    }
    return dense_gemv(S->dtype, S->n_c, S->d_coarse, b, x, s);
}

int cycle_rec(pamg_solver_s *S, int lvl, int type, int cpl, bool x_zero, hipStream_t s)
{
    Level &L = S->levels[lvl];
    Level &N = S->levels[lvl + 1];
    const int nlev = (int)S->levels.size();
    const size_t ts = tsize(S->dtype);
    PAMG_TRY(apply_smoother(S, L, L.pre, x_zero, s));
    PAMG_TRY(stream_launch(L.A, EPI_RESID, L.x, L.b, L.r, 0.0, 0.0, nullptr, s));
    PAMG_TRY(stream_launch(L.R, EPI_SET, L.r, nullptr, N.b, 0.0, 0.0, reinterpret_cast<double *>(N.x), s));
    if (lvl == nlev - 2) {
        PAMG_TRY(coarse_solve(S, N.b, N.x, s));
    } else if (type == PAMG_CYCLE_V) {
        PAMG_TRY(cycle_rec(S, lvl + 1, PAMG_CYCLE_V, 1, true, s));
    } else if (type == PAMG_CYCLE_W) {
        PAMG_TRY(cycle_rec(S, lvl + 1, PAMG_CYCLE_W, cpl, true, s));
        PAMG_TRY(cycle_rec(S, lvl + 1, PAMG_CYCLE_W, cpl, false, s));
// ... 35 lines not shown
        PAMG_HIP(hipMemcpyAsync(L.x_home, L.x, (size_t)L.n * ts, hipMemcpyDeviceToDevice, s));
        std::swap(L.x, L.xalt);
    }
    return PAMG_OK;
}

int enqueue_cycle(pamg_solver_s *S, int type, int cpl, bool check, bool x_zero, hipStream_t s)
{
    Level &L0 = S->levels[0];
    if (S->levels.size() == 1) {
        PAMG_TRY(coarse_solve(S, L0.b, L0.x, s));
    } else {
        PAMG_TRY(cycle_rec(S, 0, type, cpl, x_zero, s));
    }
    if (!check) return PAMG_OK;
    PAMG_TRY(stream_launch(L0.A, EPI_SUMSQ, L0.x, L0.b, nullptr, 0.0, 0.0, L0.A->d_partial, s));
    return reduce_partials(L0.A->d_partial, L0.A->nblk, S->d_slot, s);
}

int run_cycle(pamg_solver_s *S, int type, int cpl, hipStream_t s, bool check = true, bool x_zero = false)
{
    if (!S->use_graph || S->host_sync) return enqueue_cycle(S, type, cpl, check, x_zero, s);
    const int key = ((type * 1024 + cpl) * 2 + (check ? 1 : 0)) * 2 + (x_zero ? 1 : 0);
    auto it = S->graphs.find(key);
    if (it == S->graphs.end()) {
        hipGraph_t g = nullptr;
        PAMG_HIP(hipStreamBeginCapture(s, hipStreamCaptureModeThreadLocal));
        const int st = enqueue_cycle(S, type, cpl, check, x_zero, s);
        const hipError_t e = hipStreamEndCapture(s, &g);
        if (st != PAMG_OK) { if (g) hipGraphDestroy(g); return st; }
        if (e != hipSuccess) return (int)e;
        hipGraphExec_t ex = nullptr;
        PAMG_HIP(hipGraphInstantiate(&ex, g, nullptr, nullptr, 0));
        hipGraphDestroy(g);
        it = S->graphs.emplace(key, ex).first;
    }
    return (int)hipGraphLaunch(it->second, s);
}

int ensure_amli(pamg_solver_s *S, int cycle);

static bool sor_takes_omega(const pamg_matrix_s *A, const Smoother &sm)
{
    return sm.kind == PAMG_SMOOTH_SOR && A->R == 1 && A->flavour != PAMG_BSR && sm.sweep != PAMG_SYMMETRIC && sm.omega != 1.0;
}

static bool zero_plans_wanted(const pamg_matrix_s *A, const Smoother &pre, const Smoother &post, int l)
{
    if (A->zero_plans == 1 || (l == 0 && A->zero_plans != 2)) return false;
    if (pre.kind != PAMG_SMOOTH_GS || pre.sweep != PAMG_SYMMETRIC || pre.iterations < 1) return false;
    if (sor_takes_omega(A, post)) return false;
    return A->R == 1 && A->dtype == PAMG_F64 && A->gs_order == 1 && A->gs_mode == 0 && A->nrows >= 2;
}

int prebuild_schedules(Level &L, const Smoother &sm, bool zero)
{
    if (sm.kind == PAMG_SMOOTH_GS_NE || sm.kind == PAMG_SMOOTH_GS_NR) {
        pamg_matrix_s *Lm = sm.kind == PAMG_SMOOTH_GS_NE ? (sm.Ar ? sm.Ar : L.A) : sm.At;
        const int n = (int)Lm->nrows;
        if (n == 0) return PAMG_OK;
        if (sm.sweep != PAMG_BACKWARD) PAMG_TRY(ensure_line_schedule(Lm, 0, n, 1));
        if (sm.sweep != PAMG_FORWARD) PAMG_TRY(ensure_line_schedule(Lm, n - 1, -1, -1));
        return PAMG_OK;
    }
    const bool gs = sm.kind == PAMG_SMOOTH_GS || sm.kind == PAMG_SMOOTH_SOR || sm.kind == PAMG_SMOOTH_BLOCK_GS;
    if (!gs || L.A->nrows == 0) return PAMG_OK;
    if (sor_takes_omega(L.A, sm) && L.A->lane_merge == 0) L.A->lane_merge = 1;
    int r0, r1, rs;
    if (sm.sweep == PAMG_FORWARD || sm.sweep == PAMG_SYMMETRIC) {
        PAMG_TRY(sweep_bounds(L.A, PAMG_FORWARD, r0, r1, rs));
        PAMG_TRY(ensure_schedule(L.A, r0, r1, rs, sm.kind == PAMG_SMOOTH_BLOCK_GS));
    }
    if (sm.sweep == PAMG_BACKWARD || sm.sweep == PAMG_SYMMETRIC) {
        PAMG_TRY(sweep_bounds(L.A, PAMG_BACKWARD, r0, r1, rs));
        PAMG_TRY(ensure_schedule(L.A, r0, r1, rs, sm.kind == PAMG_SMOOTH_BLOCK_GS));
    }
    if (sm.sweep == PAMG_SYMMETRIC && sm.kind != PAMG_SMOOTH_BLOCK_GS) PAMG_TRY(ensure_sym_parts(L.A));
    if (zero) PAMG_TRY(ensure_zero_parts(L.A, true));
    return PAMG_OK;
}

struct SchedJob { pamg_matrix_s *A; int r0, r1, rs; int st; bool block_gs; int zero_dir; };

static int sched_job_run(SchedJob &j)
{
    PAMG_TRY(ensure_schedule(j.A, j.r0, j.r1, j.rs, j.block_gs));
    if (j.zero_dir < 0) return PAMG_OK;
    GsSchedule *g = nullptr;
    PAMG_TRY(get_schedule(j.A, j.r0, j.r1, j.rs, &g));
    if (!g || !g->lanem) return PAMG_OK;
    const int st = build_zero_plan(j.A, j.zero_dir);
    return st == PAMG_E_ARG ? PAMG_OK : st;
}

void sched_jobs_of(Level &L, const Smoother &sm, std::vector<SchedJob> &jobs, bool zero = false)
{
    const bool gs = sm.kind == PAMG_SMOOTH_GS || sm.kind == PAMG_SMOOTH_SOR || sm.kind == PAMG_SMOOTH_BLOCK_GS;
    if (!gs || L.A->nrows == 0) return;
    auto add = [&](int dir) {
        int r0, r1, rs;
        if (sweep_bounds(L.A, dir, r0, r1, rs)) return;
        for (const SchedJob &j : jobs) if (j.A == L.A && j.r0 == r0 && j.r1 == r1 && j.rs == rs && j.block_gs == (sm.kind == PAMG_SMOOTH_BLOCK_GS)) return;
        jobs.push_back({L.A, r0, r1, rs, PAMG_OK, sm.kind == PAMG_SMOOTH_BLOCK_GS, zero ? (dir == PAMG_BACKWARD ? 1 : 0) : -1});
    };
    if (sm.sweep == PAMG_FORWARD || sm.sweep == PAMG_SYMMETRIC) add(PAMG_FORWARD);
    if (sm.sweep == PAMG_BACKWARD || sm.sweep == PAMG_SYMMETRIC) add(PAMG_BACKWARD);
// ... 621 lines not shown

int pamg_matrix_jacobi_step(pamg_matrix_t A, const void *x_in, const void *b, void *x_out, double omega,
                            pamg_stream_t s)
{
    if (!A || !x_in || !b || !x_out) return PAMG_E_ARG;
    if (A->R != A->C || A->ncols < A->nrows) return PAMG_E_UNSUPPORTED;
    if (A->nrows == 0) return PAMG_OK;
    if (A->R > 1) return block_jacobi_step(A, PNT_JACOBI, nullptr, x_in, x_out, b, omega, (hipStream_t)s);
    return stream_launch(A, A->flavour == PAMG_BSR ? EPI_JACOBI_B : EPI_JACOBI, x_in, b, x_out, 0.0, omega,
                         nullptr, (hipStream_t)s);
}

int pamg_matrix_block_jacobi_step(pamg_matrix_t A, const void *Dinv, const void *x_in, const void *b, void *x_out,
                                  double omega, pamg_stream_t s)
{
    if (!A || !Dinv || !x_in || !b || !x_out) return PAMG_E_ARG;
    if (A->R != A->C || A->R < 2 || A->ncols < A->nrows) return PAMG_E_UNSUPPORTED;
    if (A->nrows == 0) return PAMG_OK;
    return block_jacobi_step(A, BLK_JACOBI, Dinv, x_in, x_out, b, omega, (hipStream_t)s);
}

int pamg_matrix_block_jacobi_indexed(pamg_matrix_t A, const void *Dinv, void *x, const void *b, const int32_t *idx,
                                     int64_t nidx, double omega, void *work, pamg_stream_t s)
{
    if (!A || !Dinv || !x || !b || !work || nidx < 0 || (nidx > 0 && !idx)) return PAMG_E_ARG;
    if (A->R != A->C || A->R < 2 || A->ncols != A->nrows) return PAMG_E_UNSUPPORTED;
    if (A->nrows == 0 || nidx == 0) return PAMG_OK;
    PAMG_TRY(block_jacobi_step(A, BLK_JACOBI, Dinv, x, work, b, omega, (hipStream_t)s));
    return vec_copy_indexed(A->dtype, nidx, idx, work, x, (hipStream_t)s);
}

int pamg_matrix_gauss_seidel(pamg_matrix_t A, void *x, const void *b, int sweep, double omega,
                             int iterations, pamg_stream_t s)
{
    if (!A || !x || !b || iterations < 0) return PAMG_E_ARG;
    if (sweep < PAMG_FORWARD || sweep > PAMG_SYMMETRIC) return PAMG_E_ARG;
    return gs_apply(A, x, b, sweep, omega, iterations, (hipStream_t)s);
}

int pamg_matrix_gauss_seidel_x0(pamg_matrix_t A, void *x, const void *b, int sweep, double omega,
                                int iterations, int x_is_zero, pamg_stream_t s)
{
    if (!A || !x || !b || iterations < 0) return PAMG_E_ARG;
    if (sweep < PAMG_FORWARD || sweep > PAMG_SYMMETRIC) return PAMG_E_ARG;
    return gs_apply(A, x, b, sweep, omega, iterations, (hipStream_t)s, x_is_zero != 0);
}

int pamg_matrix_gauss_seidel_correction(pamg_matrix_t A, void *x, const void *b, void *r, int iterations, pamg_stream_t s)
{
    if (!A || !x || !b || !r || iterations < 0) return PAMG_E_ARG;
    if (!square_ok(A)) return PAMG_E_ARG;
    for (int it = 0; it < iterations; ++it) {
        bool ran = false;
        PAMG_TRY(gs_sweep_correction(A, x, b, r, true, (hipStream_t)s, &ran));
        if (!ran) return PAMG_E_UNSUPPORTED;
    }
    return PAMG_OK;
}

int pamg_matrix_polynomial(pamg_matrix_t A, void *x, const void *b, void *work, const double *coeffs,
                           int ncoeffs, int iterations, int x_is_zero, pamg_stream_t s)
{
    if (!A || !x || !b || !work || iterations < 0) return PAMG_E_ARG;
    return poly_apply(A, x, b, work, coeffs, ncoeffs, iterations, x_is_zero, (hipStream_t)s);
}

int pamg_matrix_block_jacobi(pamg_matrix_t A, void *x, const void *b, void *work, const void *Dinv,
                             double omega, int iterations, pamg_stream_t s)
{
    if (!A || !x || !b || !work || iterations < 0) return PAMG_E_ARG;
    void *cur = x, *alt = work;
    PAMG_TRY(block_jacobi_pp(A, &cur, &alt, b, Dinv, omega, iterations, (hipStream_t)s));
    if (cur != x)
        PAMG_HIP(hipMemcpyAsync(x, cur, (size_t)A->nrows * tsize(A->dtype), hipMemcpyDeviceToDevice, (hipStream_t)s));
    return PAMG_OK;
}

int pamg_matrix_block_gauss_seidel(pamg_matrix_t A, void *x, const void *b, const void *Dinv, int sweep,
                                   int iterations, pamg_stream_t s)
{
    if (!A || !x || !b || iterations < 0) return PAMG_E_ARG;
    if (sweep < PAMG_FORWARD || sweep > PAMG_SYMMETRIC) return PAMG_E_ARG;
    return block_gs_apply(A, x, b, Dinv, sweep, iterations, (hipStream_t)s);
}

int pamg_solver_create(pamg_solver_t *S, int dtype)
{
    if (!S) return PAMG_E_ARG;
    if (dtype != PAMG_F64 && dtype != PAMG_F32) return PAMG_E_UNSUPPORTED;
    pamg_solver_s *p = new (std::nothrow) pamg_solver_s();
    if (!p) return PAMG_E_ALLOC;
    p->dtype = dtype;
    *S = p;
    return PAMG_OK;
}

int pamg_solver_destroy(pamg_solver_t S)
{
    if (!S) return PAMG_OK;
    drop_graphs(S);
    for (Level &L : S->levels) {
        if (L.A) L.A->borrowed--;
        if (L.P) L.P->borrowed--;
        if (L.R) L.R->borrowed--;
        hipFree(L.x); hipFree(L.xalt);
        hipFree(L.b); hipFree(L.r); hipFree(L.work); hipFree(L.amli);
        hipFree(L.pre.d_Dinv); hipFree(L.post.d_Dinv);
// ... 241 lines not shown
{
    if (!S || !fn || n_c < 1) return PAMG_E_ARG;
    if (S->finalized) return PAMG_E_STATE;
    S->coarse_host = fn; S->coarse_host_user = user;
    S->n_c = n_c; S->coarse_set = true; S->coarse_zero = false; S->coarse_relax = false;
    S->coarse_hb.assign((size_t)n_c * tsize(S->dtype), 0);
    S->coarse_hx.assign((size_t)n_c * tsize(S->dtype), 0);
    S->host_sync = true;
    return PAMG_OK;
}

int pamg_solver_set_coarse_relax(pamg_solver_t S)
{
    if (!S || S->levels.empty()) return PAMG_E_ARG;
    if (S->finalized) return PAMG_E_STATE;
    if (S->levels.back().P) return PAMG_E_STATE;
    if (S->levels.back().pre.kind == PAMG_SMOOTH_NONE) return PAMG_E_ARG;
    S->coarse_relax = true; S->coarse_set = true; S->coarse_zero = false;
    S->coarse_host = nullptr; S->coarse_host_user = nullptr;
    recompute_host_sync(S);
    S->n_c = (int)S->levels.back().n;
    return PAMG_OK;
}

int pamg_solver_finalize(pamg_solver_t S)
{
    if (!S || S->levels.empty()) return PAMG_E_ARG;
    if (S->finalized) return PAMG_OK;
    if (S->levels.back().P) return PAMG_E_STATE;
    if (!S->coarse_set || S->n_c != S->levels.back().n) return PAMG_E_STATE;
    const size_t ts = tsize(S->dtype);
    const int nlev = (int)S->levels.size();
    for (int l = 0; l < nlev; ++l) {
        Level &L = S->levels[l];
        const size_t vb = (size_t)L.n * ts;
        PAMG_TRY(dalloc(S, &L.x, vb));
        PAMG_TRY(dalloc(S, &L.xalt, vb));
        PAMG_TRY(dalloc(S, &L.b, vb));
        L.x_home = L.x;
        if (l < nlev - 1 || S->coarse_relax) {
            PAMG_TRY(dalloc(S, &L.r, vb));
            if (L.pre.kind == PAMG_SMOOTH_POLY || L.post.kind == PAMG_SMOOTH_POLY) PAMG_TRY(dalloc(S, &L.work, 3 * vb));
        }
    }
    const int nsm = S->coarse_relax ? nlev : nlev - 1;
    for (int l = 0; l < nsm; ++l) {
        Level &L = S->levels[l];
        if ((sor_takes_omega(L.A, L.pre) || sor_takes_omega(L.A, L.post)) && L.A->lane_merge == 0) L.A->lane_merge = 1;
    }
    {
        std::vector<SchedJob> jobs;
        for (int l = 0; l < nsm; ++l) {
            Level &L = S->levels[l];
            sched_jobs_of(L, L.pre, jobs, zero_plans_wanted(L.A, L.pre, L.post, l));
            sched_jobs_of(L, L.post, jobs);
        }
        PAMG_TRY(run_sched_jobs(jobs));
    }
    for (int l = 0; l < nsm; ++l) {
        Level &L = S->levels[l];
        PAMG_TRY(prebuild_schedules(L, L.pre, zero_plans_wanted(L.A, L.pre, L.post, l)));
        PAMG_TRY(prebuild_schedules(L, L.post));
    }
    PAMG_TRY(dalloc(S, (void **)&S->d_slot, 16 * sizeof(double)));
    PAMG_TRY(dalloc(S, (void **)&S->d_scratch, 1032 * sizeof(double)));
    PAMG_HIP(hipStreamCreateWithFlags(&S->own_stream, hipStreamNonBlocking));
    S->finalized = true;
    return PAMG_OK;
}

int pamg_solver_set_graph(pamg_solver_t S, int enable)
{
    if (!S) return PAMG_E_ARG;
    S->use_graph = enable != 0;
    if (!S->use_graph) drop_graphs(S);
    return PAMG_OK;
}

int pamg_solver_cycle(pamg_solver_t S, void *x, const void *b, int cycle, int cycles_per_level, pamg_stream_t s_)
{
    if (!S || !x || !b) return PAMG_E_ARG;
    if (!S->finalized) return PAMG_E_STATE;
    if (cycle < PAMG_CYCLE_V || cycle > PAMG_CYCLE_AMLI || cycles_per_level < 1 || cycles_per_level > 1023) return PAMG_E_ARG;
    hipStream_t s = s_ ? (hipStream_t)s_ : S->own_stream;
    PAMG_TRY(ensure_amli(S, cycle));
    if (!s_) PAMG_HIP(hipStreamSynchronize(nullptr));
    Level &L0 = S->levels[0];
    const size_t vb = (size_t)L0.n * tsize(S->dtype);
    PAMG_HIP(hipMemcpyAsync(L0.x, x, vb, hipMemcpyDeviceToDevice, s));
    PAMG_HIP(hipMemcpyAsync(L0.b, b, vb, hipMemcpyDeviceToDevice, s));
    PAMG_TRY(run_cycle(S, cycle, cycles_per_level, s));
    PAMG_HIP(hipMemcpyAsync(x, L0.x, vb, hipMemcpyDeviceToDevice, s));
    if (!s_) PAMG_HIP(hipStreamSynchronize(s));
    return PAMG_OK;
}

}

namespace pamg {
int solver_cycle_inline(pamg_solver_s *S, void *x, const void *b, int cycle, int cpl, hipStream_t s, bool allow_graph)
{
    if (!S || !x || !b || !s) return PAMG_E_ARG;
    if (!S->finalized) return PAMG_E_STATE;
    if (cycle == PAMG_CYCLE_AMLI) return PAMG_E_UNSUPPORTED;
    Level &L0 = S->levels[0];
    const size_t vb = (size_t)L0.n * tsize(S->dtype);
    PAMG_HIP(hipMemcpyAsync(L0.x, x, vb, hipMemcpyDeviceToDevice, s));
    PAMG_HIP(hipMemcpyAsync(L0.b, b, vb, hipMemcpyDeviceToDevice, s));
    if (allow_graph) PAMG_TRY(run_cycle(S, cycle, cpl, s, false, false));
    else PAMG_TRY(enqueue_cycle(S, cycle, cpl, false, false, s));
    PAMG_HIP(hipMemcpyAsync(x, L0.x, vb, hipMemcpyDeviceToDevice, s));
    return PAMG_OK;
}

// ... 239 lines not shown
```

pyamg_amd/multilevel.py:

```python
from __future__ import annotations

import ctypes as C
from typing import List, Optional

import numpy as np

from . import _capi as capi
from .hierarchy import HierarchySpec, SmootherSpec, SparseOp, extract

__all__ = ["DeviceMatrix", "DeviceMultilevelSolver", "TUNE_KEYS"]


TUNE_KEYS = {
    "lds_entries": 0, "max_rows": 2, "flow_cap": 3, "gs_mode": 5, "gran_cap": 6, "gran_xcd": 7, "stream_flags": 8, "gs_prof": 11, "tile_G": 12, "tile_W": 13, "tile_cap": 14,
    "tile_default": 15, "tile_D": 16, "tile_Q": 17, "tile_part": 18, "idx16": 19, "gs_cap": 20, "val8": 21, "rowgather": 22, "rowpat": 23, "gs_order": 24, "lane_L": 25, "lane_G": 26,
    "lane_wide": 27, "lane_flags": 28, "line_scan": 30, "rowmask_kz": 31, "rowmask_flags": 32, "lane_merge": 33, "lanem_ahead": 34, "lanem_rpw": 35, "lds_pad": 36, "sym_fused": 37,
    "lanem_cluster": 38, "zero_plans": 39, "zero_merge": 40, "gs_correction": 41,
}


class DeviceMatrix:

    def __init__(self, op: SparseOp):
        lib = capi.lib()
# ... 118 lines not shown
        a = (C.c_int64 * 8)()
        capi.check(capi.lib().pamg_matrix_line_info(self.handle, which, a), "pamg_matrix_line_info")
        return dict(zip(("slots_per_row", "chunks", "lines", "line_levels", "early_entries", "launch_grid", "widest_level_lines", "bytes"), list(a)))

    def kz_info(self, which=0):
        a = (C.c_int64 * 8)()
        capi.check(capi.lib().pamg_matrix_kz_info(self.handle, which, a), "pamg_matrix_kz_info")
        return dict(zip(("lanes_per_line", "slots_per_lane", "groups", "dependency_levels", "widest_level_groups", "launch_grid", "bytes"), list(a)[:7]))

    def lane_profile(self, which=0):
        n = C.c_int64(0)
        lib = capi.lib()
        capi.check(lib.pamg_matrix_lane_profile(self.handle, which, None, 0, C.byref(n)), "pamg_matrix_lane_profile")
        out = np.zeros((n.value, 4), dtype=np.int64)
        if n.value:
            capi.check(lib.pamg_matrix_lane_profile(self.handle, which, C.c_void_p(out.ctypes.data), n.value, C.byref(n)), "pamg_matrix_lane_profile")
        return out

    def tune(self, **knobs):
        unknown = [k for k in knobs if k not in TUNE_KEYS]
        if unknown:
            raise TypeError(f"tune() got an unexpected keyword argument {unknown[0]!r}")
        lib = capi.lib()
        for name, key in TUNE_KEYS.items():
            if knobs.get(name) is not None:
                capi.check(lib.pamg_matrix_tune(self.handle, key, int(knobs[name])), "pamg_matrix_tune")

    def spmv(self, mode, x, y, b=None, c=0.0, stream=None, part=None):
        if part is not None:
            capi.check(capi.lib().pamg_matrix_spmv_part(self.handle, int(part), mode, x.ptr, b.ptr if b is not None else None,
                                                        float(c), y.ptr, stream), "pamg_matrix_spmv_part")
            return
        capi.check(capi.lib().pamg_matrix_spmv(self.handle, mode, x.ptr, b.ptr if b is not None else None,
                                               float(c), y.ptr, stream), "pamg_matrix_spmv")

    def split_ranges(self, n_owned_cols: int):
        capi.check(capi.lib().pamg_matrix_split_ranges(self.handle, int(n_owned_cols)), "pamg_matrix_split_ranges")

    def resid_sumsq(self, x, b, out, stream=None):
        capi.check(capi.lib().pamg_matrix_resid_sumsq(self.handle, x.ptr, b.ptr, out.ptr, stream),
                   "pamg_matrix_resid_sumsq")

    def jacobi(self, x, b, work, omega, iterations=1, stream=None):
        capi.check(capi.lib().pamg_matrix_jacobi(self.handle, x.ptr, b.ptr, work.ptr, float(omega),
                                                 int(iterations), stream), "pamg_matrix_jacobi")

    def gauss_seidel(self, x, b, sweep="forward", omega=1.0, iterations=1, stream=None):
        capi.check(capi.lib().pamg_matrix_gauss_seidel(self.handle, x.ptr, b.ptr, capi.SWEEP[sweep],
                                                       float(omega), int(iterations), stream),
                   "pamg_matrix_gauss_seidel")

    def gauss_seidel_correction(self, x, b, r, iterations=1, stream=None):
        capi.check(capi.lib().pamg_matrix_gauss_seidel_correction(self.handle, x.ptr, b.ptr, r.ptr, int(iterations), stream), "pamg_matrix_gauss_seidel_correction")

    def gauss_seidel_x0(self, x, b, sweep="symmetric", omega=1.0, iterations=1, x_is_zero=False, stream=None):
        capi.check(capi.lib().pamg_matrix_gauss_seidel_x0(self.handle, x.ptr, b.ptr, capi.SWEEP[sweep], float(omega), int(iterations),
                                                          int(bool(x_is_zero)), stream), "pamg_matrix_gauss_seidel_x0")

    def polynomial(self, x, b, work, coefficients, iterations=1, x_is_zero=False, stream=None):
        co = np.ascontiguousarray(coefficients, dtype=np.float64)
        capi.check(capi.lib().pamg_matrix_polynomial(self.handle, x.ptr, b.ptr, work.ptr, capi.ptr(co),
                                                     co.size, int(iterations), int(bool(x_is_zero)), stream),
                   "pamg_matrix_polynomial")

    def block_jacobi(self, x, b, work, Dinv, omega, iterations=1, stream=None):
        capi.check(capi.lib().pamg_matrix_block_jacobi(self.handle, x.ptr, b.ptr, work.ptr, Dinv.ptr,
                                                       float(omega), int(iterations), stream),
                   "pamg_matrix_block_jacobi")

    def block_gauss_seidel(self, x, b, Dinv, sweep="forward", iterations=1, stream=None):
        capi.check(capi.lib().pamg_matrix_block_gauss_seidel(self.handle, x.ptr, b.ptr, Dinv.ptr,
                                                             capi.SWEEP[sweep], int(iterations), stream),
                   "pamg_matrix_block_gauss_seidel")

    def free(self):
        if getattr(self, "handle", None):
            try:
                capi._lib.pamg_matrix_destroy(self.handle)
            except Exception:
                pass
            self.handle = None

    def __del__(self):
        self.free()


def _set_smoother(lib, S, level, which, s: Optional[SmootherSpec], dtype, aux, fast=False, schwarz=None):
    if s is None or s.kind == "none":
        capi.check(lib.pamg_solver_set_smoother(S, level, which, 0, 0, 1.0, 0, None, 0, None, 1), "set_smoother")
        return
    if s.kind in ("gauss_seidel_ne", "gauss_seidel_nr", "jacobi_ne"):
        Dinv = np.ascontiguousarray(s.Dinv, dtype=dtype)
        At = None
        if s.At is not None:
            At = DeviceMatrix(s.At)
            aux.append(At)
        Ar = None
        if getattr(s, "Ar", None) is not None:
            Ar = DeviceMatrix(s.Ar)
            aux.append(Ar)
        if fast:
            for m_ in (At, Ar):
                if m_ is not None:
                    m_.tune(gs_order=1)
        capi.check(lib.pamg_solver_set_ne_smoother(S, level, which, capi.SMOOTH[s.kind], int(s.iterations), float(s.omega),
                                                   capi.SWEEP.get(s.sweep, 0), capi.ptr(Dinv), At.handle if At else None,
# ... 20 lines not shown
    if s.kind == "schwarz":
        Ar = None
        if getattr(s, "Ar", None) is not None:
            Ar = DeviceMatrix(s.Ar)
            aux.append(Ar)
        Sp, Sj = np.ascontiguousarray(s.subdomain_ptr, dtype=np.int32), np.ascontiguousarray(s.subdomain, dtype=np.int32)
        report = {"path": s.blocks_by, **(s.setup_report or {})}
        if schwarz is not None and schwarz["setup"] == "device" and s.blocks_by != "device":
            from .relaxation import _schwarz_blocks_device
            last = schwarz.get("last")
            if last is not None and last[0] == level and np.array_equal(last[1], Sj) and np.array_equal(last[2], Sp):
                Tx, Tp, report = last[3:]
            else:
                host_op = s.Ar if s.Ar is not None else schwarz["A_host"]
                Tx, Tp, report = _schwarz_blocks_device(host_op.to_scipy(), Sj, Sp, dA=Ar if Ar is not None else schwarz["A_dev"])
                schwarz["last"] = (level, Sj, Sp, Tx, Tp, report)
        else:
            Tp, Tx = np.ascontiguousarray(s.inv_subblock_ptr, dtype=np.int32), np.ascontiguousarray(s.inv_subblock, dtype=dtype)
        if schwarz is not None:
            schwarz["reports"].setdefault(level, {})["pre" if which == 0 else "post"] = report
        capi.check(lib.pamg_solver_set_schwarz_smoother(S, level, which, int(s.iterations), capi.SWEEP.get(s.sweep, 0),
                                                        Ar.handle if Ar else None, Sp.size - 1, capi.ptr(Sp), capi.ptr(Sj),
                                                        capi.ptr(Tp), capi.ptr(Tx)),
                   "pamg_solver_set_schwarz_smoother")
        return
    if s.kind in ("cf_block_jacobi", "fc_block_jacobi"):
        F = np.ascontiguousarray(s.Fpts, dtype=np.int32)
        Cp = np.ascontiguousarray(s.Cpts, dtype=np.int32)
        Dinv = np.ascontiguousarray(s.Dinv, dtype=dtype)
        capi.check(lib.pamg_solver_set_cf_block_smoother(S, level, which, capi.SMOOTH[s.kind], int(s.iterations),
                                                         int(s.f_iterations), int(s.c_iterations), float(s.omega),
                                                         capi.ptr(Dinv), int(s.blocksize), capi.ptr(F), F.size,
                                                         capi.ptr(Cp), Cp.size),
                   f"pamg_solver_set_cf_block_smoother({s.kind})")
        return
    coeffs = None
    ncoef = 0
    if s.kind == "polynomial":
        coeffs = np.ascontiguousarray(s.coefficients, dtype=np.float64)
        ncoef = coeffs.size
    Dinv = None
    if s.kind in ("block_jacobi", "block_gauss_seidel"):
        Dinv = np.ascontiguousarray(s.Dinv, dtype=dtype)
    capi.check(lib.pamg_solver_set_smoother(
        S, level, which, capi.SMOOTH[s.kind], int(s.iterations), float(s.omega),
        capi.SWEEP.get(s.sweep, 0), capi.ptr(coeffs), ncoef, capi.ptr(Dinv), int(s.blocksize)),
        f"pamg_solver_set_smoother({s.kind})")


class DeviceMultilevelSolver:

    def __init__(self, ml, device: Optional[int] = None, graph: bool = True, autotune: Optional[bool] = None,
                 level_tune=None, order: Optional[str] = None, strict: bool = True, renumber: Optional[bool] = None,
                 schwarz_setup: str = "reference"):
        import os
        self.fallback = None
        if schwarz_setup not in ("reference", "device"):
            raise ValueError("schwarz_setup must be 'reference' or 'device'")
        self.schwarz_setup, self._schwarz_reports = schwarz_setup, {}
        if not strict:
            try:
                self.__init__(ml, device=device, graph=graph, autotune=autotune, level_tune=level_tune, order=order, strict=True, renumber=renumber,
                              schwarz_setup=schwarz_setup)
                return
            except NotImplementedError as e:
                if isinstance(ml, HierarchySpec) or not hasattr(ml, "solve"):
                    raise
                import warnings
                warnings.warn(f"pyamg_amd: this hierarchy is not on the device path ({e}); strict=False hands every call to the wrapped "
                              "solver on the host", RuntimeWarning, stacklevel=2)
                self.free()
                self.fallback, self.ml, self.spec, self.handle = ml, ml, None, None
                self.renumbered, self.renumber_seconds = [], 0.0
                self.order = order or "fast"
                A0 = ml.levels[0].A
                self.dtype, self.shape = np.dtype(A0.dtype), tuple(A0.shape)
                self.A, self._mats, self._aux = [], [], []
                self.symmetric_smoothing = getattr(ml, "symmetric_smoothing", False)
                return
        if autotune is None:
            autotune = os.environ.get("PAMG_AUTOTUNE", "1") != "0"
        if order is None:
            order = os.environ.get("PAMG_GS_ORDER", "fast")
        if order not in ("fast", "exact"):
            raise ValueError("order must be 'fast' or 'exact'")
        self.order = order
        self._device, self._graph, self._autotune, self._level_tune = device, graph, autotune, level_tune
        self.ml = None if isinstance(ml, HierarchySpec) else ml
        self.spec = ml if isinstance(ml, HierarchySpec) else extract(ml, schwarz_setup)
        lib = capi.lib()
        if renumber is None:
            renumber = os.environ.get("PAMG_RENUMBER", "0") != "0"
        dev_spec, self.renumbered, self.renumber_seconds = self.spec, [], 0.0
        if renumber:
            import time
            from .renumber import renumber_levels
            t0 = time.perf_counter()
            dev_spec, orders = renumber_levels(self.spec)
            self.renumbered, self.renumber_seconds = sorted(orders), time.perf_counter() - t0
        if device is not None:
            capi.check(lib.pamg_set_device(int(device)), "pamg_set_device")
        self.dtype = np.dtype(self.spec.dtype)
        self.shape = tuple(self.spec.levels[0].A.shape)
        self._mats: List[DeviceMatrix] = []
        self._aux: List[DeviceMatrix] = []
        self.A: List[DeviceMatrix] = []
        h = C.c_void_p()
        capi.check(lib.pamg_solver_create(C.byref(h), capi.dtype_code(self.dtype)), "pamg_solver_create")
        self.handle = h
        nlev = len(self.spec.levels)
        ops = []
        for i, L in enumerate(dev_spec.levels):
            ops += [L.A] + ([L.P, L.R] if i < nlev - 1 else [])

        cur = C.c_int(0)
        capi.check(lib.pamg_get_device(C.byref(cur)), "pamg_get_device")
        cur = int(cur.value)

        def ship(op):
            capi.check(lib.pamg_set_device(cur), "pamg_set_device")
            return DeviceMatrix(op)

        nthreads = int(os.environ.get("PAMG_UPLOAD_THREADS", "8"))
        if nthreads > 1 and len(ops) > 1:
            from concurrent.futures import ThreadPoolExecutor
            with ThreadPoolExecutor(max_workers=min(nthreads, len(ops))) as ex:
                shipped = list(ex.map(ship, ops))
        else:
            shipped = [ship(op) for op in ops]
        self._mats = list(shipped)
        shipped = iter(shipped)
        for i, L in enumerate(dev_spec.levels):
            A = next(shipped)
            P = next(shipped) if i < nlev - 1 else None
            R = next(shipped) if i < nlev - 1 else None
            self.A.append(A)
            if autotune:
                gs_level = i < nlev - 1 and any(s is not None and s.kind in ("gauss_seidel", "sor", "block_gauss_seidel")
                                                for s in (L.pre, L.post))
                A.autotune(allow_cap=not gs_level)
                for m in (P, R):
                    if m is not None:
                        m.autotune(allow_cap=True)
            if order == "fast":
                A.tune(gs_order=1)
            if level_tune is not None:
                kw = level_tune(i) if callable(level_tune) else level_tune
                if kw:
                    A.tune(**kw)
            capi.check(lib.pamg_solver_add_level(h, A.handle, P.handle if P else None, R.handle if R else None),
                       "pamg_solver_add_level")
            if i < nlev - 1:
                sw = {"setup": schwarz_setup, "A_host": L.A, "A_dev": A, "reports": self._schwarz_reports}
                _set_smoother(lib, h, i, 0, L.pre, self.dtype, self._aux, fast=order == "fast", schwarz=sw)
                _set_smoother(lib, h, i, 1, L.post, self.dtype, self._aux, fast=order == "fast", schwarz=sw)
        n_c = self.spec.levels[-1].A.shape[0]
        if self.spec.coarse_kind == "relax":
            _set_smoother(lib, h, nlev - 1, 0, self.spec.coarse_smoother, self.dtype, self._aux, fast=order == "fast",
                          schwarz={"setup": schwarz_setup, "A_host": dev_spec.levels[-1].A, "A_dev": self.A[-1], "reports": self._schwarz_reports})
            capi.check(lib.pamg_solver_set_coarse_relax(h), "set_coarse_relax")
        elif self.spec.coarse_kind == "host":
            cs, A_c = self.spec.coarse_host
            dt = self.dtype

            def _coarse(_user, b_ptr, x_ptr, n):
                try:
                    bh = np.ctypeslib.as_array(C.cast(b_ptr, C.POINTER(C.c_double if dt == np.float64 else C.c_float)), shape=(int(n),))
                    xh = np.ctypeslib.as_array(C.cast(x_ptr, C.POINTER(C.c_double if dt == np.float64 else C.c_float)), shape=(int(n),))
                    xh[:] = np.ravel(cs(A_c, np.array(bh, dtype=dt))).astype(dt, copy=False)
                    return 0
                except Exception:
                    import traceback
                    traceback.print_exc()
                    return 1
            self._coarse_cb = C.CFUNCTYPE(C.c_int, C.c_void_p, C.c_void_p, C.c_void_p, C.c_int64)(_coarse)
            capi.check(lib.pamg_solver_set_coarse_host(h, C.cast(self._coarse_cb, C.c_void_p), None, n_c), "set_coarse_host")
        elif self.spec.coarse_kind == "zero":
            capi.check(lib.pamg_solver_set_coarse_dense(h, None, n_c), "set_coarse")
        else:
            M = np.ascontiguousarray(self.spec.coarse_op, dtype=self.dtype)
            capi.check(lib.pamg_solver_set_coarse_dense(h, capi.ptr(M), n_c), "set_coarse")
        capi.check(lib.pamg_solver_set_graph(h, int(bool(graph))), "set_graph")
        capi.check(lib.pamg_solver_finalize(h), "pamg_solver_finalize")
        self.symmetric_smoothing = getattr(self.ml, "symmetric_smoothing", False)
        self._xd = capi.DeviceArray(self.shape[0], self.dtype)
        self._bd = capi.DeviceArray(self.shape[0], self.dtype)

    @property
    def levels(self):
        return self.spec.levels if self.spec is not None else self.fallback.levels

    def __repr__(self):
        if self.fallback is not None:
            return "DeviceMultilevelSolver (strict=False: not on the device path, calls go to the wrapped solver)\n" + repr(self.fallback)
        lines = ["DeviceMultilevelSolver (MI355X resident)", f"Number of Levels:     {len(self.spec.levels)}",
                 f"Coarse Solver:        {self.spec.coarse_name}", "  level   unknowns     nonzeros"]
        tot = sum(L.A.nnz for L in self.spec.levels)
        for i, L in enumerate(self.spec.levels):
            lines.append(f"{i:>6} {L.A.shape[0]:>11} {L.A.nnz:>12} [{100 * L.A.nnz / max(tot, 1):2.2f}%]")
        return "\n".join(lines) + "\n"

    def _need_device(self, what):
# ... 281 lines not shown
```

Measured before the change: 96.26 cycles/s.

## Add dense block-triangular-inverse Gauss-Seidel path for coarse AMG levels

Adds a new smoother path that precomputes explicit dense inverses of the lower and upper triangular factors within row blocks, with a growth check that declines unstable inverses. Symmetric Gauss-Seidel is then applied as a sequence of per-block sparse off-block updates plus dense triangular matvecs. The path is selected automatically on coarse levels that use symmetric GS pre- and post-smoothing and pass size and memory limits. The aim is to swap the dependency-bound sparse triangular sweep for bandwidth-friendly dense matvecs. The cost is extra setup time, more device memory and a launch count that grows with the number of blocks.

After: 102.4 cycles/s (median of 6 runs). 1.06x the previous value.

```diff
diff --git a/include/pyamg_amd.h b/include/pyamg_amd.h
--- a/include/pyamg_amd.h
+++ b/include/pyamg_amd.h
@@ -390,6 +390,8 @@
                                 int iterations, int x_is_zero, pamg_stream_t s);
 int pamg_matrix_sym_info(pamg_matrix_t A, int64_t info[9]);
 int pamg_matrix_gauss_seidel_correction(pamg_matrix_t A, void *x, const void *b, void *r, int iterations, pamg_stream_t s);
+int pamg_matrix_dense_tri(pamg_matrix_t A, int mode, int block_rows);
+int pamg_matrix_dense_tri_info(pamg_matrix_t A, int64_t info[16], double *growth);
 int pamg_matrix_polynomial(pamg_matrix_t A, void *x, const void *b, void *work,
                            const double *coeffs, int ncoeffs, int iterations, int x_is_zero,
                            pamg_stream_t s);
diff --git a/pyamg_amd/_build.py b/pyamg_amd/_build.py
--- a/pyamg_amd/_build.py
+++ b/pyamg_amd/_build.py
@@ -10,8 +10,8 @@
 PKG = Path(__file__).resolve().parent
 CSRC = PKG / "csrc"
 LIB = PKG / "libpyamg_amd.so"
-SOURCES = ["pamg_matrix.hip", "pamg_solver.hip", "pamg_capi.hip", "pamg_setup.hip", "pamg_schwarz.hip", "pamg_dist.hip", "pamg_aggregate.hip", "pamg_lane.hip", "pamg_line.hip", "pamg_kz.hip", "pamg_blane.hip", "pamg_block.hip", "pamg_renumber.hip", "pamg_krylov.hip", "pamg_schwarz_setup.hip", "pamg_classical.hip", "pamg_air.hip", "pamg_evolution.hip", "pamg_energy.hip"]
-HEADERS = ["pamg_common.h", "pamg_kernels.h", "pamg_tile_kernels.h", "pamg_tile_plan.h", "pamg_lane_plan.h", "pamg_lanem_plan.h", "pamg_schwarz_plan.h", "pamg_line_plan.h", "pamg_kz_plan.h", "pamg_blane_plan.h", "pamg_spg_plan.h", "pamg_stream_plan.h", "pamg_rowmask_map.h", "pamg_plan_vec.h", "pamg_host_threads.h", "pamg_dense_pinv.h", "pamg_classical.h", "pamg_air.h", "pamg_jacobi_svd.h", "pamg_evolution.h", "pamg_energy.h", "pamg_host_call.h", "pamg_wave.h", "pamg_sweep_host.h", "amg_core_bind.cpp", "../../include/pyamg_amd.h"]
+SOURCES = ["pamg_matrix.hip", "pamg_solver.hip", "pamg_capi.hip", "pamg_setup.hip", "pamg_schwarz.hip", "pamg_dist.hip", "pamg_aggregate.hip", "pamg_lane.hip", "pamg_line.hip", "pamg_kz.hip", "pamg_blane.hip", "pamg_block.hip", "pamg_renumber.hip", "pamg_krylov.hip", "pamg_schwarz_setup.hip", "pamg_classical.hip", "pamg_air.hip", "pamg_evolution.hip", "pamg_energy.hip", "pamg_dtri.hip"]
+HEADERS = ["pamg_common.h", "pamg_kernels.h", "pamg_tile_kernels.h", "pamg_tile_plan.h", "pamg_lane_plan.h", "pamg_lanem_plan.h", "pamg_schwarz_plan.h", "pamg_line_plan.h", "pamg_kz_plan.h", "pamg_blane_plan.h", "pamg_spg_plan.h", "pamg_stream_plan.h", "pamg_rowmask_map.h", "pamg_plan_vec.h", "pamg_host_threads.h", "pamg_dense_pinv.h", "pamg_classical.h", "pamg_air.h", "pamg_jacobi_svd.h", "pamg_evolution.h", "pamg_energy.h", "pamg_host_call.h", "pamg_wave.h", "pamg_sweep_host.h", "pamg_dtri_plan.h", "amg_core_bind.cpp", "../../include/pyamg_amd.h"]
 FLAGS = ["--offload-arch=gfx950", "-O3", "-std=c++17", "-fPIC", "-ffp-contract=off",
          "-fno-fast-math", "-Wall", "-Wno-unused-function", "-Wno-unused-value", "-Wno-unused-result"]
 
diff --git a/pyamg_amd/_capi.py b/pyamg_amd/_capi.py
--- a/pyamg_amd/_capi.py
+++ b/pyamg_amd/_capi.py
@@ -180,6 +180,8 @@
     f("pamg_matrix_gauss_seidel", _vp, _vp, _vp, _i, _d, _i, _vp)
     f("pamg_matrix_gauss_seidel_x0", _vp, _vp, _vp, _i, _d, _i, _i, _vp)
     f("pamg_matrix_gauss_seidel_correction", _vp, _vp, _vp, _vp, _i, _vp)
+    f("pamg_matrix_dense_tri", _vp, _i, _i)
+    f("pamg_matrix_dense_tri_info", _vp, P(C.c_int64), P(C.c_double))
     f("pamg_matrix_sym_info", _vp, P(C.c_int64))
     f("pamg_matrix_polynomial", _vp, _vp, _vp, _vp, _vp, _i, _i, _i, _vp)
     f("pamg_matrix_block_jacobi", _vp, _vp, _vp, _vp, _vp, _d, _i, _vp)
diff --git a/pyamg_amd/csrc/pamg_common.h b/pyamg_amd/csrc/pamg_common.h
--- a/pyamg_amd/csrc/pamg_common.h
+++ b/pyamg_amd/csrc/pamg_common.h
@@ -130,6 +130,8 @@
     int64_t n_local = 0, n_global = 0, n_publish = 0, max_step_entries = 0;
     size_t bytes = 0;
 };
+
+struct DtriSched;
 
 struct LineSchedule {
     int start = 0, stop = 0, step = 0;
@@ -240,6 +242,14 @@
     long long zero_plan_launches = 0;
     int gs_correction = 0;
     long long correction_launches = 0;
+    int dtri_mode = 0;
+    int dtri_block_rows = 0;
+    struct pamg::DtriSched *dtri = nullptr;
+    bool dtri_unfit = false;
+    bool dtri_declined_growth = false;
+    double dtri_growth = 0.0;
+    size_t dtri_bytes = 0;
+    long long dtri_zero_launches = 0, dtri_correction_launches = 0;
     size_t bytes = 0;
 };
 
@@ -363,6 +373,20 @@
 int gs_sweep_zero_pair(pamg_matrix_s *A, void *x, const void *b, hipStream_t s, bool *ran);
 int gs_sweep_correction(pamg_matrix_s *A, void *x, const void *b, void *r, bool force, hipStream_t s, bool *ran);
 constexpr int64_t GS_CORRECTION_MIN_ROWS = 16384;
+constexpr int64_t ONE_XCD_MAX_ROWS = 8192;
+constexpr int64_t DTRI_AUTO_RATIO = 16;
+constexpr int64_t DTRI_MAX_BYTES = (int64_t)2 << 30;
+bool dtri_form_ok(const pamg_matrix_s *A);
+bool dtri_auto_eligible(const pamg_matrix_s *A);
+int build_dtri_part(pamg_matrix_s *A);
+void free_dtri_part(struct DtriSched *t);
+size_t dtri_part_bytes(const pamg_matrix_s *A);
+int dtri_sym_launch(pamg_matrix_s *A, void *x, const void *b, bool acc, hipStream_t s);
+int dtri_info(const pamg_matrix_s *A, int64_t *info, double *growth);
+bool dtri_claims(const pamg_matrix_s *A, bool sweeps, bool automatic);
+int ensure_dtri(pamg_matrix_s *A, bool sweeps, bool automatic);
+void matrix_drop_dtri(pamg_matrix_s *A);
+int gs_sweep_dtri(pamg_matrix_s *A, void *x, const void *b, void *r, bool x_zero, hipStream_t s, bool *ran);
 int sym_fill_sentinels(void *p, int64_t n);
 int sweep_error(pamg_matrix_s *A, bool *error);
 inline size_t tsize(int dtype) { return dtype == PAMG_F64 ? 8 : 4; }
diff --git a/pyamg_amd/csrc/pamg_dtri.hip b/pyamg_amd/csrc/pamg_dtri.hip
--- /dev/null
+++ b/pyamg_amd/csrc/pamg_dtri.hip
@@ -0,0 +1,268 @@
+#include "pamg_common.h"
+#include "pamg_dtri_plan.h"
+#include "pamg_wave.h"
+#include "pamg_sweep_host.h"
+
+namespace pamg {
+
+struct DtriSched {
+    int n = 0, B = 0, nb = 0;
+    int *d_Lp = nullptr, *d_Lj = nullptr, *d_Up = nullptr, *d_Uj = nullptr;
+    double *d_Lx = nullptr, *d_Ux = nullptr;
+    double *d_W[2] = {nullptr, nullptr};
+    double *d_t = nullptr, *d_y = nullptr, *d_dy = nullptr, *d_z = nullptr;
+    int64_t *d_woff = nullptr;
+    unsigned long long *d_growth = nullptr;
+    std::vector<int64_t> woff;
+    int64_t tri_bytes = 0, off_block = 0;
+    double growth = 0.0;
+    float inverse_ms = 0.f;
+    size_t bytes = 0;
+};
+
+namespace {
+
+constexpr int DTRI_L = 16;
+
+__global__ __launch_bounds__(BLK) void dtri_inverse_kernel(const int *__restrict__ Ap, const int *__restrict__ Aj, const double *__restrict__ Ax,
+                                                          const double *__restrict__ diag, int n, int B, const int64_t *__restrict__ woff,
+                                                          double *W, int dir)
+{
+    const int k = blockIdx.y, lo = k * B, hi = min(lo + B, n), m = hi - lo;
+    const int j0 = blockIdx.x * BLK;
+    if (j0 >= m) return;
+    const int j = j0 + threadIdx.x;
+    double *Wk = W + woff[k];
+    for (int i = j0; i < m; ++i) {
+        if (j > i) continue;
+        const int gi = dir ? hi - 1 - i : lo + i;
+        const int64_t ro = dtri_row_off(i);
+        double s = i == j ? 1.0 : 0.0;
+        for (int p = Ap[gi]; p < Ap[gi + 1]; ++p) {
+            const int gc = Aj[p];
+            if (gc < lo || gc >= hi) continue;
+            const int c = dir ? hi - 1 - gc : gc - lo;
+            if (c >= i || c < j) continue;
+            s = s - Ax[p] * Wk[dtri_row_off(c) + j];
+        }
+        Wk[ro + j] = s / diag[gi];
+        if (i == j && !(i & 1)) Wk[ro + i + 1] = 0.0;
+    }
+}
+
+__global__ __launch_bounds__(BLK) void dtri_growth_kernel(const double *__restrict__ diag, int n, int B, const int64_t *__restrict__ woff,
+                                                         const double *__restrict__ W, int dir, unsigned long long *out)
+{
+    const int64_t r = ((int64_t)blockIdx.x * BLK + threadIdx.x) >> 6;
+    const int lane = threadIdx.x & 63;
+    if (r >= n) return;
+    const int k = (int)(r / B), lo = k * B, hi = min(lo + B, n), i = (int)r - lo;
+    const double *Wr = W + woff[k] + dtri_row_off(i);
+    double s = 0.0;
+    for (int j = lane; j <= i; j += 64) s += fabs(Wr[j]) * fabs(diag[dir ? hi - 1 - j : lo + j]);
+    s = seg_allreduce<64>(s);
+    if (!(s <= 1.79e308)) s = INFINITY;
+    if (lane == 0) atomicMax(out, (unsigned long long)__double_as_longlong(s));
+}
+
+template <bool BWD>
+__global__ __launch_bounds__(BLK) void gs_dtri_sparse_kernel(const int *__restrict__ Sp, const int *__restrict__ Sj, const double *__restrict__ Sx,
+                                                            const double *__restrict__ rhs, const double *__restrict__ v, double *__restrict__ t,
+                                                            int lo, int hi)
+{
+    const int m = hi - lo;
+    const int l = (blockIdx.x * BLK + threadIdx.x) / DTRI_L, lane = threadIdx.x & (DTRI_L - 1);
+    const bool live = l < m;
+    const int g = live ? (BWD ? hi - 1 - l : lo + l) : lo;
+    const int p0 = live ? Sp[g] : 0, p1 = live ? Sp[g + 1] : 0;
+    double s = 0.0;
+    for (int p = p0 + lane; p < p1; p += DTRI_L) s += Sx[p] * v[Sj[p]];
+    s = seg_allreduce<DTRI_L>(s);
+    if (live && lane == 0) t[l] = rhs[g] - s;
+}
+
+template <bool BWD>
+__global__ __launch_bounds__(BLK) void gs_dtri_dense_kernel(const double *__restrict__ W, const double *__restrict__ t, int tglobal,
+                                                           const double *__restrict__ diag, double *__restrict__ o1, double *o2, int acc,
+                                                           int lo, int hi)
+{
+    typedef double d2 __attribute__((ext_vector_type(2)));
+    static_assert(BLK == 256, "four waves per workgroup");
+    __shared__ double part[4][2];
+    const int m = hi - lo;
+    const int w = blockIdx.x, lane = threadIdx.x & 63, wave = threadIdx.x >> 6;
+    const int i0 = w, i1 = m - 1 - w;
+    const int nd0 = (i0 + 2) >> 1, nd1 = i0 == i1 ? 0 : (i1 + 2) >> 1;
+    const d2 *W0 = reinterpret_cast<const d2 *>(W + dtri_row_off(i0)), *W1 = reinterpret_cast<const d2 *>(W + dtri_row_off(i1));
+    double s0 = 0.0, s1 = 0.0;
+#pragma unroll 4
+    for (int q = threadIdx.x; q < nd0 + nd1; q += BLK) {
+        const bool second = q >= nd0;
+        const int qq = second ? q - nd0 : q, i = second ? i1 : i0, j = 2 * qq;
+        const d2 wv = __builtin_nontemporal_load((second ? W1 : W0) + qq);
+        double v = wv.x * t[tglobal ? (BWD ? hi - 1 - j : lo + j) : j];
+        if (j + 1 <= i) v += wv.y * t[tglobal ? (BWD ? hi - 2 - j : lo + j + 1) : j + 1];
+        if (second) s1 += v; else s0 += v;
+    }
+    s0 = seg_allreduce<64>(s0);
+    s1 = seg_allreduce<64>(s1);
+    if (lane == 0) { part[wave][0] = s0; part[wave][1] = s1; }
+    __syncthreads();
+    if (threadIdx.x < (i0 == i1 ? 1 : 2)) {
+        const int h = threadIdx.x, i = h ? i1 : i0;
+        const double s = (part[0][h] + part[1][h]) + (part[2][h] + part[3][h]);
+        const int g = BWD ? hi - 1 - i : lo + i;
+        o1[g] = s;
+        if (BWD) o2[g] = acc ? o2[g] + s : s;
+        else o2[g] = diag[g] * s;
+    }
+}
+
+}
+
+void free_dtri_part(DtriSched *t)
+{
+    if (!t) return;
+    hipFree(t->d_Lp); hipFree(t->d_Lj); hipFree(t->d_Lx); hipFree(t->d_Up); hipFree(t->d_Uj); hipFree(t->d_Ux);
+    hipFree(t->d_W[0]); hipFree(t->d_W[1]); hipFree(t->d_t); hipFree(t->d_y); hipFree(t->d_dy); hipFree(t->d_z);
+    hipFree(t->d_woff); hipFree(t->d_growth);
+    delete t;
+}
+
+bool dtri_form_ok(const pamg_matrix_s *A)
+{
+    return A->dtype == PAMG_F64 && A->R == 1 && A->C == 1 && A->nrows == A->ncols && A->nrows >= 1 && A->nrows < INT32_MAX &&
+           A->gs_order == 1 && A->gs_mode == 0 && !A->gs_prof && A->d_Ax && A->d_diag && !A->h_Ap.empty();
+}
+
+int dtri_block_rows(const pamg_matrix_s *A) { return A->dtri_block_rows > 0 ? A->dtri_block_rows : DTRI_BLOCK_ROWS; }
+
+int64_t dtri_tri_bytes(int64_t n, int B)
+{
+    const int64_t full = n / B, rest = n - full * B;
+    return 8 * (full * dtri_tri_slots(B) + dtri_tri_slots(rest));
+}
+
+bool dtri_auto_eligible(const pamg_matrix_s *A)
+{
+    if (!dtri_form_ok(A) || A->nrows <= ONE_XCD_MAX_ROWS || A->dtri_unfit) return false;
+    const int64_t tri = dtri_tri_bytes(A->nrows, dtri_block_rows(A));
+    return tri <= DTRI_AUTO_RATIO * (12 * A->nnz + 4 * (A->nrows + 1)) && 2 * tri <= DTRI_MAX_BYTES;
+}
+
+int build_dtri_part(pamg_matrix_s *A)
+{
+    if (A->dtri || A->dtri_unfit) return A->dtri ? PAMG_OK : PAMG_E_ARG;
+    auto decline = [&](bool growth) { A->dtri_unfit = true; A->dtri_declined_growth = growth; return PAMG_E_ARG; };
+    if (!dtri_form_ok(A)) return decline(false);
+    const int n = (int)A->nrows, B = dtri_block_rows(A);
+    if (2 * dtri_tri_bytes(n, B) > DTRI_MAX_BYTES || (n + B - 1) / B > 65535) return decline(false);
+    PhaseTimer pt_("build_dtri_part", A->nnz);
+    std::vector<double> hAx((size_t)A->nnz + 1);
+    if (A->nnz) PAMG_HIP(hipMemcpy(hAx.data(), A->d_Ax, (size_t)A->nnz * sizeof(double), hipMemcpyDeviceToHost));
+    DtriPlan P;
+    if (build_dtri_plan(n, A->h_Ap.data(), A->h_Aj.data(), hAx.data(), B, P) != DTRI_OK) return decline(false);
+    hAx = std::vector<double>();
+    DtriSched *t = new (std::nothrow) DtriSched();
+    if (!t) return PAMG_E_ALLOC;
+    t->n = n; t->B = B; t->nb = P.nb; t->woff = P.woff; t->off_block = P.off_block_entries();
+    const size_t wb = (size_t)P.woff[(size_t)P.nb] * sizeof(double), vb = ((size_t)n + 8) * sizeof(double);
+    t->tri_bytes = 2 * (int64_t)wb;
+    int st = device_upload(&t->d_Lp, P.Lp.data(), P.Lp.size() * sizeof(int), &t->bytes);
+    if (!st) st = device_upload(&t->d_Lj, P.Lj.data(), P.Lj.size() * sizeof(int), &t->bytes);
+    if (!st) st = device_upload(&t->d_Lx, P.Lx.data(), P.Lx.size() * sizeof(double), &t->bytes);
+    if (!st) st = device_upload(&t->d_Up, P.Up.data(), P.Up.size() * sizeof(int), &t->bytes);
+    if (!st) st = device_upload(&t->d_Uj, P.Uj.data(), P.Uj.size() * sizeof(int), &t->bytes);
+    if (!st) st = device_upload(&t->d_Ux, P.Ux.data(), P.Ux.size() * sizeof(double), &t->bytes);
+    if (!st) st = device_upload(&t->d_woff, P.woff.data(), P.woff.size() * sizeof(int64_t), &t->bytes);
+    if (!st) st = device_upload(&t->d_growth, nullptr, 2 * sizeof(unsigned long long), &t->bytes);
+    for (int d = 0; d < 2 && !st; ++d) st = device_upload(&t->d_W[d], nullptr, wb, &t->bytes);
+    if (!st) st = device_upload(&t->d_t, nullptr, ((size_t)B + 8) * sizeof(double), &t->bytes);
+    if (!st) st = device_upload(&t->d_y, nullptr, vb, &t->bytes);
+    if (!st) st = device_upload(&t->d_dy, nullptr, vb, &t->bytes);
+    if (!st) st = device_upload(&t->d_z, nullptr, vb, &t->bytes);
+    if (!st) st = (int)hipMemset(t->d_growth, 0, 2 * sizeof(unsigned long long));
+    hipEvent_t e0 = nullptr, e1 = nullptr;
+    if (!st) st = (int)hipEventCreate(&e0);
+    if (!st) st = (int)hipEventCreate(&e1);
+    if (!st) {
+        const int m = std::min(B, n);
+        hipEventRecord(e0, 0);
+        for (int d = 0; d < 2; ++d)
+            hipLaunchKernelGGL(dtri_inverse_kernel, dim3((m + BLK - 1) / BLK, P.nb), dim3(BLK), 0, 0, (const int *)A->d_Ap, (const int *)A->d_Aj,
+                               (const double *)A->d_Ax, (const double *)A->d_diag, n, B, (const int64_t *)t->d_woff, t->d_W[d], d);
+        hipEventRecord(e1, 0);
+        const unsigned gg = (unsigned)(((int64_t)n * 64 + BLK - 1) / BLK);
+        for (int d = 0; d < 2; ++d)
+            hipLaunchKernelGGL(dtri_growth_kernel, dim3(gg), dim3(BLK), 0, 0, (const double *)A->d_diag, n, B, (const int64_t *)t->d_woff,
+                               (const double *)t->d_W[d], d, t->d_growth + d);
+        st = (int)hipGetLastError();
+    }
+    unsigned long long gbits[2] = {0, 0};
+    if (!st) st = (int)hipMemcpy(gbits, t->d_growth, sizeof(gbits), hipMemcpyDeviceToHost);
+    if (!st) hipEventElapsedTime(&t->inverse_ms, e0, e1);
+    if (e0) hipEventDestroy(e0);
+    if (e1) hipEventDestroy(e1);
+    if (st) { free_dtri_part(t); return st; }
+    double g[2];
+    memcpy(g, gbits, sizeof(g));
+    t->growth = std::max(g[0], g[1]);
+    A->dtri_growth = t->growth;
+    if (!(t->growth <= DTRI_GROWTH_CAP)) { free_dtri_part(t); return decline(true); }
+    A->dtri = t;
+    return PAMG_OK;
+}
+
+size_t dtri_part_bytes(const pamg_matrix_s *A) { return A->dtri ? A->dtri->bytes : 0; }
+
+int dtri_launches(const DtriSched *t) { return 4 * t->nb - 2; }
+
+int dtri_sym_launch(pamg_matrix_s *A, void *x_, const void *b_, bool acc, hipStream_t s)
+{
+    DtriSched *t = A->dtri;
+    if (!t) return PAMG_E_STATE;
+    double *x = (double *)x_;
+    const double *b = (const double *)b_, *diag = (const double *)A->d_diag;
+    const int n = t->n, B = t->B, nb = t->nb;
+    auto grids = [&](int m, unsigned &gs, unsigned &gd) {
+        gs = (unsigned)(((int64_t)m * DTRI_L + BLK - 1) / BLK);
+        gd = (unsigned)((m + 1) / 2);
+    };
+    for (int k = 0; k < nb; ++k) {
+        const int lo = k * B, hi = std::min(lo + B, n);
+        unsigned gs, gd;
+        grids(hi - lo, gs, gd);
+        if (k > 0)
+            hipLaunchKernelGGL((gs_dtri_sparse_kernel<false>), dim3(gs), dim3(BLK), 0, s, (const int *)t->d_Lp, (const int *)t->d_Lj, (const double *)t->d_Lx,
+                               b, (const double *)t->d_y, t->d_t, lo, hi);
+        hipLaunchKernelGGL((gs_dtri_dense_kernel<false>), dim3(gd), dim3(BLK), 0, s, (const double *)(t->d_W[0] + t->woff[(size_t)k]),
+                           k > 0 ? (const double *)t->d_t : b, k > 0 ? 0 : 1, diag, t->d_y, t->d_dy, 0, lo, hi);
+    }
+    for (int k = nb - 1; k >= 0; --k) {
+        const int lo = k * B, hi = std::min(lo + B, n);
+        unsigned gs, gd;
+        grids(hi - lo, gs, gd);
+        if (k < nb - 1)
+            hipLaunchKernelGGL((gs_dtri_sparse_kernel<true>), dim3(gs), dim3(BLK), 0, s, (const int *)t->d_Up, (const int *)t->d_Uj, (const double *)t->d_Ux,
+                               (const double *)t->d_dy, (const double *)t->d_z, t->d_t, lo, hi);
+        hipLaunchKernelGGL((gs_dtri_dense_kernel<true>), dim3(gd), dim3(BLK), 0, s, (const double *)(t->d_W[1] + t->woff[(size_t)k]),
+                           k < nb - 1 ? (const double *)t->d_t : (const double *)t->d_dy, k < nb - 1 ? 0 : 1, diag, t->d_z, x, acc ? 1 : 0, lo, hi);
+    }
+    return (int)hipGetLastError();
+}
+
+int dtri_info(const pamg_matrix_s *A, int64_t *info, double *growth)
+{
+    for (int i = 0; i < 16; ++i) info[i] = 0;
+    const DtriSched *t = A->dtri;
+    if (t) {
+        info[0] = 1; info[1] = t->nb; info[2] = t->B; info[3] = t->tri_bytes; info[4] = t->off_block;
+        info[9] = (int64_t)(1e3 * (double)t->inverse_ms); info[11] = dtri_launches(t); info[12] = (int64_t)t->bytes;
+    }
+    info[5] = A->dtri_zero_launches; info[6] = A->dtri_correction_launches;
+    info[7] = dtri_auto_eligible(A) ? 1 : 0; info[8] = A->dtri_declined_growth ? 1 : 0; info[10] = A->dtri_mode;
+    if (growth) *growth = A->dtri_growth;
+    return PAMG_OK;
+}
+
+}
diff --git a/pyamg_amd/csrc/pamg_dtri_plan.h b/pyamg_amd/csrc/pamg_dtri_plan.h
--- /dev/null
+++ b/pyamg_amd/csrc/pamg_dtri_plan.h
@@ -0,0 +1,143 @@
+#pragma once
+#include <algorithm>
+#include <cmath>
+#include <cstdint>
+#include <vector>
+
+#if defined(__HIPCC__)
+#define PAMG_DTRI_HD __host__ __device__ __forceinline__
+#else
+#define PAMG_DTRI_HD inline
+#endif
+
+namespace pamg {
+
+constexpr double DTRI_GROWTH_CAP = 1e3;
+constexpr int DTRI_BLOCK_ROWS = 2048;
+constexpr int DTRI_MAX_BLOCK_ROWS = 8192;
+
+enum : int { DTRI_OK = 0, DTRI_E_SHAPE = 1, DTRI_E_DIAGONAL = 2, DTRI_E_GROWTH = 3 };
+
+PAMG_DTRI_HD int64_t dtri_row_off(int64_t i) { const int64_t p = i >> 1; return (i & 1) ? 2 * (p + 1) * (p + 1) : 2 * p * (p + 1); }
+inline int64_t dtri_tri_slots(int64_t m) { return dtri_row_off(m); }
+
+struct DtriPlan {
+    int n = 0, B = 0, nb = 0;
+    std::vector<int> Lp, Lj, Up, Uj;
+    std::vector<double> Lx, Ux;
+    std::vector<double> diag;
+    std::vector<int64_t> woff;
+    int lo(int k) const { return k * B; }
+    int hi(int k) const { return (int)std::min<int64_t>((int64_t)(k + 1) * B, n); }
+    int64_t off_block_entries() const { return (int64_t)Lj.size() + (int64_t)Uj.size(); }
+};
+
+inline int build_dtri_plan(int n, const int *Ap, const int *Aj, const double *Ax, int B, DtriPlan &P)
+{
+    if (n < 1 || B < 1) return DTRI_E_SHAPE;
+    P = DtriPlan();
+    P.n = n; P.B = B; P.nb = (n + B - 1) / B;
+    P.diag.assign((size_t)n, 0.0);
+    P.Lp.assign((size_t)n + 1, 0);
+    P.Up.assign((size_t)n + 1, 0);
+    for (int i = 0; i < n; ++i) {
+        const int lo = (i / B) * B, hi = (int)std::min<int64_t>((int64_t)lo + B, n);
+        int nd = 0, cl = 0, cu = 0;
+        for (int p = Ap[i]; p < Ap[i + 1]; ++p) {
+            const int j = Aj[p];
+            if (j < 0 || j >= n) return DTRI_E_SHAPE;
+            if (j == i) { ++nd; P.diag[(size_t)i] = Ax[p]; }
+            cl += j < lo; cu += j >= hi;
+        }
+        const double d = P.diag[(size_t)i];
+        if (nd != 1 || !(d != 0.0) || !std::isfinite(d)) return DTRI_E_DIAGONAL;
+        P.Lp[(size_t)i + 1] = P.Lp[(size_t)i] + cl;
+        P.Up[(size_t)i + 1] = P.Up[(size_t)i] + cu;
+    }
+    P.Lj.resize((size_t)P.Lp[(size_t)n]); P.Lx.resize((size_t)P.Lp[(size_t)n]);
+    P.Uj.resize((size_t)P.Up[(size_t)n]); P.Ux.resize((size_t)P.Up[(size_t)n]);
+    for (int i = 0; i < n; ++i) {
+        const int lo = (i / B) * B, hi = (int)std::min<int64_t>((int64_t)lo + B, n);
+        int ql = P.Lp[(size_t)i], qu = P.Up[(size_t)i];
+        for (int p = Ap[i]; p < Ap[i + 1]; ++p) {
+            const int j = Aj[p];
+            if (j < lo) { P.Lj[(size_t)ql] = j; P.Lx[(size_t)ql] = Ax[p]; ++ql; }
+            else if (j >= hi) { P.Uj[(size_t)qu] = j; P.Ux[(size_t)qu] = Ax[p]; ++qu; }
+        }
+    }
+    P.woff.assign((size_t)P.nb + 1, 0);
+    for (int k = 0; k < P.nb; ++k) P.woff[(size_t)k + 1] = P.woff[(size_t)k] + dtri_tri_slots(P.hi(k) - P.lo(k));
+    return DTRI_OK;
+}
+
+inline void dtri_host_inverse(const DtriPlan &P, const int *Ap, const int *Aj, const double *Ax, int k, int dir, double *W)
+{
+    const int lo = P.lo(k), hi = P.hi(k), m = hi - lo;
+    for (int64_t q = 0; q < dtri_tri_slots(m); ++q) W[q] = 0.0;
+    for (int j = 0; j < m; ++j)
+        for (int i = j; i < m; ++i) {
+            const int gi = dir ? hi - 1 - i : lo + i;
+            double s = i == j ? 1.0 : 0.0;
+            for (int p = Ap[gi]; p < Ap[gi + 1]; ++p) {
+                const int gc = Aj[p];
+                if (gc < lo || gc >= hi) continue;
+                const int c = dir ? hi - 1 - gc : gc - lo;
+                if (c >= i || c < j) continue;
+                s = s - Ax[p] * W[dtri_row_off(c) + j];
+            }
+            W[dtri_row_off(i) + j] = s / P.diag[(size_t)gi];
+        }
+}
+
+inline double dtri_host_growth(const DtriPlan &P, int k, int dir, const double *W)
+{
+    const int lo = P.lo(k), hi = P.hi(k), m = hi - lo;
+    double g = 0.0;
+    for (int i = 0; i < m; ++i) {
+        double s = 0.0;
+        for (int j = 0; j <= i; ++j) s += std::fabs(W[dtri_row_off(i) + j]) * std::fabs(P.diag[(size_t)(dir ? hi - 1 - j : lo + j)]);
+        if (!std::isfinite(s)) s = INFINITY;
+        g = std::max(g, s);
+    }
+    return g;
+}
+
+inline void dtri_host_apply(const DtriPlan &P, const double *Wf, const double *Wb, const double *b, double *x, bool acc)
+{
+    const int n = P.n;
+    std::vector<double> t((size_t)P.B), y((size_t)n, 0.0), dy((size_t)n, 0.0), z((size_t)n, 0.0);
+    for (int k = 0; k < P.nb; ++k) {
+        const int lo = P.lo(k), m = P.hi(k) - lo;
+        for (int l = 0; l < m; ++l) {
+            double s = 0.0;
+            for (int p = P.Lp[(size_t)(lo + l)]; p < P.Lp[(size_t)(lo + l) + 1]; ++p) s += P.Lx[(size_t)p] * y[(size_t)P.Lj[(size_t)p]];
+            t[(size_t)l] = b[lo + l] - s;
+        }
+        const double *W = Wf + P.woff[(size_t)k];
+        for (int l = 0; l < m; ++l) {
+            double s = 0.0;
+            for (int j = 0; j <= l; ++j) s += W[dtri_row_off(l) + j] * t[(size_t)j];
+            y[(size_t)(lo + l)] = s;
+            dy[(size_t)(lo + l)] = P.diag[(size_t)(lo + l)] * s;
+        }
+    }
+    for (int k = P.nb - 1; k >= 0; --k) {
+        const int hi = P.hi(k), m = hi - P.lo(k);
+        for (int l = 0; l < m; ++l) {
+            const int g = hi - 1 - l;
+            double s = 0.0;
+            for (int p = P.Up[(size_t)g]; p < P.Up[(size_t)g + 1]; ++p) s += P.Ux[(size_t)p] * z[(size_t)P.Uj[(size_t)p]];
+            t[(size_t)l] = dy[(size_t)g] - s;
+        }
+        const double *W = Wb + P.woff[(size_t)k];
+        for (int l = 0; l < m; ++l) {
+            const int g = hi - 1 - l;
+            double s = 0.0;
+            for (int j = 0; j <= l; ++j) s += W[dtri_row_off(l) + j] * t[(size_t)j];
+            z[(size_t)g] = s;
+            x[g] = acc ? x[g] + s : s;
+        }
+    }
+}
+
+}
diff --git a/pyamg_amd/csrc/pamg_lane.hip b/pyamg_amd/csrc/pamg_lane.hip
--- a/pyamg_amd/csrc/pamg_lane.hip
+++ b/pyamg_amd/csrc/pamg_lane.hip
@@ -1179,7 +1179,7 @@
 
 static bool lanem_one_xcd(const pamg_matrix_s *A, const GsSchedule *g, const LaneMSched *t)
 {
-    return !t->cluster && (A->gran_xcd == 1 || (A->gran_xcd == 0 && lane_one_xcd(A, g) && A->nrows <= 8192));
+    return !t->cluster && (A->gran_xcd == 1 || (A->gran_xcd == 0 && lane_one_xcd(A, g) && A->nrows <= ONE_XCD_MAX_ROWS));
 }
 
 static int lanem_want_grid(const pamg_matrix_s *A, const LaneMSched *t, int cap, int cus)
diff --git a/pyamg_amd/csrc/pamg_matrix.hip b/pyamg_amd/csrc/pamg_matrix.hip
--- a/pyamg_amd/csrc/pamg_matrix.hip
+++ b/pyamg_amd/csrc/pamg_matrix.hip
@@ -10,6 +10,7 @@
 #include "pamg_tile_kernels.h"
 #include "pamg_tile_plan.h"
 #include "pamg_stream_plan.h"
+#include "pamg_dtri_plan.h"
 
 using namespace pamg;
 
@@ -821,6 +822,7 @@
         if (l) free_line_schedule(l);
     }
     matrix_drop_zero_plans(A);
+    matrix_drop_dtri(A);
     matrix_drop_point_twin(A);
 }
 
@@ -1436,6 +1438,66 @@
     if (st == PAMG_E_UNSUPPORTED) st = lanem_zero_pair_launch(A, gf, gb, x, r, true, s);
     if (st != PAMG_OK) return st;
     A->correction_launches++;
+    *ran = true;
+    return PAMG_OK;
+}
+
+bool dtri_claims(const pamg_matrix_s *A, bool sweeps, bool automatic)
+{
+    if (!A || !sweeps || A->dtri_mode == 1 || A->dtri_unfit || !dtri_form_ok(A)) return false;
+    return A->dtri_mode == 2 || (automatic && dtri_auto_eligible(A));
+}
+
+void matrix_drop_dtri(pamg_matrix_s *A)
+{
+    if (!A) return;
+    A->dtri_unfit = A->dtri_declined_growth = false;
+    if (!A->dtri) return;
+    free_dtri_part(A->dtri);
+    A->dtri = nullptr;
+    std::lock_guard<std::mutex> lk(g_sched_mu);
+    A->bytes -= std::min(A->bytes, A->dtri_bytes);
+    A->dtri_bytes = 0;
+}
+
+int ensure_dtri(pamg_matrix_s *A, bool sweeps, bool automatic)
+{
+    if (!A) return PAMG_OK;
+    if (!dtri_claims(A, sweeps, automatic)) {
+        if (A->dtri) { const bool unfit = A->dtri_unfit, grew = A->dtri_declined_growth; matrix_drop_dtri(A); A->dtri_unfit = unfit; A->dtri_declined_growth = grew; }
+        return PAMG_OK;
+    }
+    if (A->dtri) return PAMG_OK;
+    const int st = build_dtri_part(A);
+    if (st == PAMG_E_ARG) return PAMG_OK;
+    if (st != PAMG_OK) return st;
+    std::lock_guard<std::mutex> lk(g_sched_mu);
+    A->dtri_bytes = dtri_part_bytes(A);
+    A->bytes += A->dtri_bytes;
+    return PAMG_OK;
+}
+
+int gs_sweep_dtri(pamg_matrix_s *A, void *x, const void *b, void *r, bool x_zero, hipStream_t s, bool *ran)
+{
+    *ran = false;
+    if (A->dtri_mode == 1 || !dtri_form_ok(A)) return PAMG_OK;
+    if (!x_zero && (!r || A->gs_correction == 1)) return PAMG_OK;
+    if (!A->dtri) {
+        if (A->dtri_mode != 2 || A->dtri_unfit) return PAMG_OK;
+        hipStreamCaptureStatus cs = hipStreamCaptureStatusNone;
+        PAMG_HIP(hipStreamIsCapturing(s, &cs));
+        if (cs != hipStreamCaptureStatusNone) return PAMG_OK;
+        PAMG_TRY(ensure_dtri(A, true, false));
+        if (!A->dtri) return PAMG_OK;
+    }
+    if (x_zero) {
+        PAMG_TRY(dtri_sym_launch(A, x, b, false, s));
+        A->dtri_zero_launches++;
+    } else {
+        PAMG_TRY(stream_launch(A, EPI_RESID, x, b, r, 0.0, 0.0, nullptr, s));
+        PAMG_TRY(dtri_sym_launch(A, x, r, true, s));
+        A->dtri_correction_launches++;
+    }
     *ran = true;
     return PAMG_OK;
 }
@@ -1908,6 +1970,7 @@
     for (int k = 0; k < 4; ++k) pamg::free_line_schedule(A->ls[k]);
     hipFree(A->d_sym_hf[0]); hipFree(A->d_sym_hf[1]); hipFree(A->d_sym_hb); hipFree(A->d_sym_sync);
     pamg::free_zero_plans(A);
+    pamg::free_dtri_part(A->dtri);
     if (A->point_twin) pamg_matrix_destroy(A->point_twin);
     delete A;
     return PAMG_OK;
@@ -2074,6 +2137,7 @@
         case DROP_LANES:
             matrix_drop_point_twin(A);
             matrix_drop_zero_plans(A);
+            matrix_drop_dtri(A);
             for (GsSchedule *g : A->gs) {
                 if (!g) continue;
                 g->lane_unfit = g->lanem_unfit = g->blane_unfit = g->line_unfit = false;
@@ -2093,6 +2157,7 @@
         case REPLAN:
             for (int k = 0; k < 4; ++k) { if (A->gs[k]) A->bytes -= A->gs[k]->bytes; free_schedule(A->gs[k]); A->gs[k] = nullptr; }
             matrix_drop_zero_plans(A);
+            matrix_drop_dtri(A);
             matrix_drop_point_twin(A);
             return replan(A);
     }
@@ -2111,6 +2176,7 @@
     if (A->borrowed > 0 && !(t && (t->flags & HELD_OK))) return PAMG_E_STATE;
     if (!t || !t->accepts(value)) return PAMG_E_ARG;
     A->*(t->field) = tune_stored(t->store, value);
+    if (A->dtri && !pamg::dtri_form_ok(A)) pamg::matrix_drop_dtri(A);
     return tune_effect(A, t->effect, value);
 }
 
@@ -2290,6 +2356,22 @@
     return PAMG_OK;
 }
 
+int pamg_matrix_dense_tri(pamg_matrix_t A, int mode, int block_rows)
+{
+    if (!A || mode < 0 || mode > 2 || block_rows < 0 || block_rows > pamg::DTRI_MAX_BLOCK_ROWS) return PAMG_E_ARG;
+    if (A->borrowed > 0) return PAMG_E_STATE;
+    if (mode != A->dtri_mode || block_rows != A->dtri_block_rows) pamg::matrix_drop_dtri(A);
+    A->dtri_mode = mode;
+    A->dtri_block_rows = block_rows;
+    return PAMG_OK;
+}
+
+int pamg_matrix_dense_tri_info(pamg_matrix_t A, int64_t info[16], double *growth)
+{
+    if (!A || !info) return PAMG_E_ARG;
+    return pamg::dtri_info(A, info, growth);
+}
+
 int pamg_matrix_lanem_levels(pamg_matrix_t A, int which, int64_t *out, int64_t capacity, int64_t *count)
 {
     if (!A || !count || which < 0 || which > 3) return PAMG_E_ARG;
diff --git a/pyamg_amd/csrc/pamg_solver.hip b/pyamg_amd/csrc/pamg_solver.hip
--- a/pyamg_amd/csrc/pamg_solver.hip
+++ b/pyamg_amd/csrc/pamg_solver.hip
@@ -93,6 +93,8 @@
     if (sweep == PAMG_SYMMETRIC) {
         for (int it = 0; it < its; ++it) {
             bool ran = false;
+            PAMG_TRY(gs_sweep_dtri(A, x, b, r, x_zero && it == 0, s, &ran));
+            if (ran) continue;
             if (r && !(x_zero && it == 0)) PAMG_TRY(gs_sweep_correction(A, x, b, r, false, s, &ran));
             if (ran) continue;
             PAMG_TRY(gs_sweep_symmetric(A, x, b, x_zero && it == 0, s, &ran));
@@ -312,6 +314,7 @@
         L.A->tile_default = 0;
         PAMG_TRY(sym_reset(L.A));
         matrix_drop_zero_plans(L.A);
+        matrix_drop_dtri(L.A);
         for (Smoother *sm : {&L.pre, &L.post}) {
             if (sm->At) sm->At->gs_mode = 1;
             if (sm->Ar) sm->Ar->gs_mode = 1;
@@ -453,6 +456,10 @@
     if (sor_takes_omega(A, post)) return false;
     return A->R == 1 && A->dtype == PAMG_F64 && A->gs_order == 1 && A->gs_mode == 0 && A->nrows >= 2;
 }
+
+static bool dtri_sym_gs(const Smoother &sm) { return sm.kind == PAMG_SMOOTH_GS && sm.sweep == PAMG_SYMMETRIC && sm.iterations >= 1; }
+static bool dtri_sweeps(const Smoother &pre, const Smoother &post) { return dtri_sym_gs(pre) || dtri_sym_gs(post); }
+static bool dtri_automatic(const Smoother &pre, const Smoother &post, int l) { return l >= 1 && dtri_sym_gs(pre) && dtri_sym_gs(post); }
 
 int prebuild_schedules(Level &L, const Smoother &sm, bool zero)
 {
@@ -1180,7 +1187,8 @@
     if (!square_ok(A)) return PAMG_E_ARG;
     for (int it = 0; it < iterations; ++it) {
         bool ran = false;
-        PAMG_TRY(gs_sweep_correction(A, x, b, r, true, (hipStream_t)s, &ran));
+        PAMG_TRY(gs_sweep_dtri(A, x, b, r, false, (hipStream_t)s, &ran));
+        if (!ran) PAMG_TRY(gs_sweep_correction(A, x, b, r, true, (hipStream_t)s, &ran));
         if (!ran) return PAMG_E_UNSUPPORTED;
     }
     return PAMG_OK;
@@ -1528,14 +1536,15 @@
         std::vector<SchedJob> jobs;
         for (int l = 0; l < nsm; ++l) {
             Level &L = S->levels[l];
-            sched_jobs_of(L, L.pre, jobs, zero_plans_wanted(L.A, L.pre, L.post, l));
+            sched_jobs_of(L, L.pre, jobs, zero_plans_wanted(L.A, L.pre, L.post, l) && !dtri_claims(L.A, dtri_sweeps(L.pre, L.post), dtri_automatic(L.pre, L.post, l)));
             sched_jobs_of(L, L.post, jobs);
         }
         PAMG_TRY(run_sched_jobs(jobs));
     }
     for (int l = 0; l < nsm; ++l) {
         Level &L = S->levels[l];
-        PAMG_TRY(prebuild_schedules(L, L.pre, zero_plans_wanted(L.A, L.pre, L.post, l)));
+        PAMG_TRY(ensure_dtri(L.A, dtri_sweeps(L.pre, L.post), dtri_automatic(L.pre, L.post, l)));
+        PAMG_TRY(prebuild_schedules(L, L.pre, zero_plans_wanted(L.A, L.pre, L.post, l) && !L.A->dtri));
         PAMG_TRY(prebuild_schedules(L, L.post));
     }
     PAMG_TRY(dalloc(S, (void **)&S->d_slot, 16 * sizeof(double)));
diff --git a/pyamg_amd/multilevel.py b/pyamg_amd/multilevel.py
--- a/pyamg_amd/multilevel.py
+++ b/pyamg_amd/multilevel.py
@@ -194,6 +194,18 @@
 
     def gauss_seidel_correction(self, x, b, r, iterations=1, stream=None):
         capi.check(capi.lib().pamg_matrix_gauss_seidel_correction(self.handle, x.ptr, b.ptr, r.ptr, int(iterations), stream), "pamg_matrix_gauss_seidel_correction")
+
+    def dense_tri(self, mode, block_rows=0):
+        capi.check(capi.lib().pamg_matrix_dense_tri(self.handle, int(mode), int(block_rows)), "pamg_matrix_dense_tri")
+
+    def dense_tri_info(self):
+        a = (C.c_int64 * 16)()
+        gr = C.c_double(0.0)
+        capi.check(capi.lib().pamg_matrix_dense_tri_info(self.handle, a, C.byref(gr)), "pamg_matrix_dense_tri_info")
+        d = dict(zip(("built", "blocks", "block_rows", "bytes", "off_block_entries", "zero_launches", "correction_launches", "auto_eligible",
+                      "declined_by_growth", "inverse_us", "mode", "kernel_launches", "resident_bytes"), (int(v) for v in a)))
+        d["growth"] = gr.value
+        return d
 
     def gauss_seidel_x0(self, x, b, sweep="symmetric", omega=1.0, iterations=1, x_is_zero=False, stream=None):
         capi.check(capi.lib().pamg_matrix_gauss_seidel_x0(self.handle, x.ptr, b.ptr, capi.SWEEP[sweep], float(omega), int(iterations),
@@ -320,7 +332,7 @@
 
     def __init__(self, ml, device: Optional[int] = None, graph: bool = True, autotune: Optional[bool] = None,
                  level_tune=None, order: Optional[str] = None, strict: bool = True, renumber: Optional[bool] = None,
-                 schwarz_setup: str = "reference"):
+                 schwarz_setup: str = "reference", dense_tri=None):
         import os
         self.fallback = None
         if schwarz_setup not in ("reference", "device"):
@@ -329,7 +341,7 @@
         if not strict:
             try:
                 self.__init__(ml, device=device, graph=graph, autotune=autotune, level_tune=level_tune, order=order, strict=True, renumber=renumber,
-                              schwarz_setup=schwarz_setup)
+                              schwarz_setup=schwarz_setup, dense_tri=dense_tri)
                 return
             except NotImplementedError as e:
                 if isinstance(ml, HierarchySpec) or not hasattr(ml, "solve"):
@@ -416,6 +428,10 @@
                 kw = level_tune(i) if callable(level_tune) else level_tune
                 if kw:
                     A.tune(**kw)
+            if dense_tri is False:
+                A.dense_tri(1)
+            elif dense_tri is not None and dense_tri.get(i):
+                A.dense_tri(**dense_tri[i])
             capi.check(lib.pamg_solver_add_level(h, A.handle, P.handle if P else None, R.handle if R else None),
                        "pamg_solver_add_level")
             if i < nlev - 1:
```
